# eora-ai/torchok

Hardware: AMD Instinct MI355X
Metric: images/sec (node) ResNet-50 224px bs256/GPU; step p50 ms (higher is better)
Workload: dtype bf16

## Files before the change

### include/tok.h

```cpp
#ifndef TOK_H_
#define TOK_H_

#include <stddef.h>
#include <stdint.h>

#ifdef __cplusplus
extern "C" {
#endif

typedef enum tok_status {
  TOK_OK = 0,
  TOK_ERR_INVALID = -1,
  TOK_ERR_LAUNCH = -2,
  TOK_ERR_WORKSPACE = -3
} tok_status;

typedef enum tok_dtype { TOK_F32 = 0, TOK_F16 = 1, TOK_BF16 = 2 } tok_dtype;

typedef struct tok_conv_desc {
  int32_t n, h, w, c;
  int32_t k;
  int32_t r, s;
  int32_t p, q;
  int32_t stride, pad;
  int32_t s_pad;
} tok_conv_desc;

const char* tok_last_error(void);
int tok_version(void);


int tok_nchw_to_nhwc_bf16(const void* src, int src_dtype, int n, int c, int h, int w,
                          void* dst, int c_pad, void* stream);
int tok_cast_f32_bf16(const float* src, void* dst, size_t count, void* stream);
int tok_cast_bf16_f32(const void* src, float* dst, float scale, size_t count, void* stream);
int tok_pack_weight_fwd(const float* src, int k, int r, int s, int c,
                        void* dst, int k_pad, int s_pad, int c_pad, void* stream);
int tok_pack_weight_dgrad(const float* src, int k, int r, int s, int c,
                          void* dst, int k_pad, int c_pad, void* stream);

int tok_pack_weight_both(const float* src, int k, int r, int s, int c, void* dst_fwd, int k_pad,
                         int s_pad, int c_pad, void* dst_dgrad, void* stream);

typedef struct tok_pack_item {
  const float* src;
  void* dst_fwd;
  void* dst_dgrad;
  int32_t k, r, s, c, k_pad, s_pad, c_pad;
  int32_t block_start;
} tok_pack_item;
int tok_pack_item_blocks(const tok_pack_item* item );
int tok_pack_weights_batched(const tok_pack_item* items_dev, int n_items, int total_blocks, void* stream);


int tok_conv_fwd_stat_rows(const tok_conv_desc* d);
int tok_conv_fwd(const tok_conv_desc* d, const void* x, const void* w, const float* bias,
                 void* y, float* stats, void* stream);
int tok_conv_dgrad(const tok_conv_desc* d, const void* dy, const void* w_dgrad, void* dx,
                   int accumulate, void* stream);
int tok_conv_dgrad_stat_rows(const tok_conv_desc* d);
int tok_conv_dgrad_bnstats(const tok_conv_desc* d, const void* dy, const void* w_dgrad, void* dx,
                           int accumulate, const void* bn_y, const uint8_t* bn_mask, float* partial,
                           void* stream);
int tok_bn_gram_finalize(const float* Z, const float* zsum, const float* w, int64_t count, int p, int k,
                         const float* gamma, const float* beta, float* running_mean, float* running_var,
                         int64_t* num_batches_tracked, float momentum, float eps, float* mean, float* rstd,
                         float* scale, float* shift, float* wz ,
                         void* stream);
int tok_conv_fwd_bn_apply(const tok_conv_desc* d, const void* x, const void* w, const float* scale, const float* shift,
                          const void* shortcut , int relu, void* out, uint8_t* mask ,
                          void* stream);
int tok_conv_dgrad_maskstore(const tok_conv_desc* d, const void* dy, const void* w_dgrad, void* dx, int accumulate,
                             const uint8_t* mask, float* partial, void* stream);
int tok_relu_mask_reduce(const void* dout, const uint8_t* mask, int64_t m, int c, void* dz, float* partial, void* stream);
int tok_bn3_bwd_prepare(const float* G, const float* w, const float* wz, const float* zsum, const float* partial, int rows,
                        int64_t count, int p, int k, const float* gamma, const float* mean, const float* rstd,
                        float* dgamma, float* dbeta, int param_accumulate, float* coef, float* dw, int dw_accumulate,
                        void* wa, void* wb, float* cvec, float* ws ,
                        void* stream);
size_t tok_bn3_bwd_prepare_ws_floats(int p, int k);
int tok_conv_dgrad_bias(const tok_conv_desc* d, const void* dy, const void* w_dgrad, const float* bias, void* dx,
                        int accumulate, const void* bn_y, const uint8_t* bn_mask, float* partial, void* stream);
int tok_subsample2_fwd(const void* x, int n, int h, int w, int c, void* out, void* stream);
int tok_subsample2_bwd(const void* dsub, int n, int h, int w, int c, void* dx, int accumulate, void* stream);
int tok_conv_dgrad_subacc_ok(const tok_conv_desc* d);
int tok_conv_dgrad_subacc(const tok_conv_desc* d, const void* dy, const void* w_dgrad, void* dx, const void* dsub,
                          const void* bn_y , const uint8_t* mask ,
                          float* partial , int mask_store, void* stream);
int tok_conv_dgrad2_ok(const tok_conv_desc* d1, const tok_conv_desc* d2);
int tok_conv_dgrad2(const tok_conv_desc* d1, const void* dy1, const void* w1_dgrad, const tok_conv_desc* d2, const void* dy2,
                    const void* w2_dgrad, const float* bias , void* dx, int accumulate,
                    const void* bn_y , const uint8_t* bn_mask , float* partial ,
                    void* stream);
size_t tok_conv_wgrad_ws_bytes(const tok_conv_desc* d);
int tok_conv_wgrad(const tok_conv_desc* d, const void* x, const void* dy, float* dw,
                   int k_real, int c_real, void* ws, size_t ws_bytes, int accumulate,
                   void* stream);
int tok_conv_wgrad_bias_ok(const tok_conv_desc* d);
size_t tok_conv_wgrad_bias_ws_bytes(const tok_conv_desc* d);
int tok_conv_wgrad_bias(const tok_conv_desc* d, const void* x, const void* dy, float* dw, int k_real, int c_real,
                        void* ws, size_t ws_bytes, int accumulate, float* dbias, int bias_accumulate, void* stream);


int tok_bn_finalize(const float* stats, int rows, int64_t count, int c, int c_real,
                    const float* gamma, const float* beta,
                    float* running_mean, float* running_var, int64_t* nbt,
                    float momentum, float eps,
                    float* mean, float* rstd, float* scale, float* shift, void* stream);
int tok_bn_eval_coeffs(const float* gamma, const float* beta, const float* running_mean,
                       const float* running_var, float eps, int c, int c_real,
                       float* scale, float* shift, void* stream);
int tok_bn_stats_rows(int64_t m, int c);
int tok_bn_stats(const void* y, int64_t m, int c, float* stats, void* stream);
int tok_bn_act_fwd(const void* y, const float* scale, const float* shift,
                   const void* shortcut, int relu, void* out, uint8_t* mask, int64_t m, int c,
                   void* stream);
void* tok_event_create(void);
int tok_event_destroy(void* ev);
int tok_next_launch_event(void* ev);
int tok_stream_wait_event(void* stream, void* ev);
int tok_bn_act_fwd_colsum_rows(int64_t m, int c);
int tok_bn_act_fwd_colsum(const void* y, const float* scale, const float* shift, const void* shortcut, int relu, void* out,
                          uint8_t* mask, int64_t m, int c, float* partial, void* stream);
int tok_bn_bwd_rows(int64_t m, int c);
int tok_bn_bwd_reduce(const void* dout, const void* y, const uint8_t* mask,
                      const float* scale, const float* shift,
                      const float* mean, const float* rstd, int relu,
                      int64_t m, int c, float* partial, void* stream);
int tok_bn_bwd_finalize(const float* partial, int rows, int64_t m, int c, int c_real,
                        const float* gamma, const float* mean, const float* rstd,
                        float* dgamma, float* dbeta, float* coef, int accumulate, int dzy_form,
                        void* stream);
int tok_bn_bwd_apply(const void* dout, const void* y, const uint8_t* mask,
                     const float* scale, const float* shift, const float* coef, int relu,
                     void* dy, void* dshortcut, int dshortcut_accumulate,
                     int64_t m, int c, void* stream);
int tok_bn_hswish_fwd(const void* y, const float* scale, const float* shift, void* out, int64_t m, int c, void* stream);
int tok_bn_hswish_bwd_reduce(const void* dout, const void* y, const float* scale, const float* shift, const float* mean,
                             const float* rstd, int64_t m, int c, float* partial, void* stream);
int tok_bn_hswish_bwd_apply(const void* dout, const void* y, const float* scale, const float* shift, const float* coef,
                            void* dy, int64_t m, int c, void* stream);
int tok_bn_relu6_fwd(const void* y, const float* scale, const float* shift, void* out, int64_t m, int c, void* stream);
int tok_bn_relu6_bwd_reduce(const void* dout, const void* y, const float* scale, const float* shift, const float* mean,
                            const float* rstd, int64_t m, int c, float* partial, void* stream);
int tok_bn_relu6_bwd_apply(const void* dout, const void* y, const float* scale, const float* shift, const float* coef,
                           void* dy, int64_t m, int c, void* stream);


int tok_maxpool3x3s2_fwd(const void* x, void* y, uint8_t* argmax, int n, int h, int w, int c,
                         void* stream);
int tok_maxpool3x3s2_bwd(const void* dy, const uint8_t* argmax, void* dx, int accumulate,
                         int n, int h, int w, int c, void* stream);
int tok_avgpool2x2_fwd(const void* x, void* y, int n, int h, int w, int c, void* stream);
int tok_avgpool2x2_bwd(const void* dy, void* dx, int accumulate, int n, int h, int w, int c, void* stream);
int tok_gap_fwd(const void* x, void* y, int n, int hw, int c, void* stream);
int tok_gap_bwd(const void* dy, void* dx, int accumulate, int n, int hw, int c, void* stream);
int tok_global_pool_fwd(const void* x, void* y, int* argmax, int n, int hw, int c, int ldy, int mode, void* stream);
int tok_global_pool_bwd(const void* dy, const int* argmax, void* dx, int accumulate, int n, int hw, int c, int ldy,
                        int mode, void* stream);

int tok_colsum(const void* dy, int64_t m, int n_pad, int n_real, float* out, int accumulate,
               void* stream);

#define TOK_CE_LOSS_FLOATS 2050
int tok_softmax_ce_fwd(const void* logits, const int64_t* target, int rows, int classes, int ld,
                       int64_t ignore_index, float* lse, float* row_loss,
                       float* loss , void* stream);
int tok_softmax_ce_bwd(const void* logits, const int64_t* target, const float* lse,
                       const float* loss, const float* gscale, int rows, int classes, int ld,
                       int64_t ignore_index, void* dlogits, void* stream);

int tok_softmax_ce_smooth_fwd(const void* logits, const int64_t* target, int rows, int classes, int ld,
                              int64_t ignore_index, float label_smoothing, float* lse, float* row_loss,
                              float* loss, void* stream);
int tok_softmax_ce_smooth_bwd(const void* logits, const int64_t* target, const float* lse, const float* loss,
                              const float* gscale, int rows, int classes, int ld, int64_t ignore_index,
                              float label_smoothing, void* dlogits, void* stream);

int tok_upsample_ce_serves(int classes, int ld);
int tok_upsample_ce_fwd(const void* low, int n, int hs, int ws, int classes, int ld, int hd, int wd, const int64_t* target,
// ... 278 lines not shown
```

### torchok_amd/_C.py

```python
import ctypes
import os
from ctypes import POINTER, Structure, c_char_p, c_float, c_int, c_int32, c_int64, c_size_t, c_void_p

_HERE = os.path.dirname(os.path.abspath(__file__))
LIB_PATH = os.environ.get('TOK_LIB') or os.path.join(_HERE, 'lib', 'libtok_gfx950.so')

TOK_F32, TOK_F16, TOK_BF16 = 0, 1, 2
TOK_CE_LOSS_FLOATS = 2050


class ConvDesc(Structure):
    _fields_ = [('n', c_int32), ('h', c_int32), ('w', c_int32), ('c', c_int32),
                ('k', c_int32), ('r', c_int32), ('s', c_int32),
                ('p', c_int32), ('q', c_int32),
                ('stride', c_int32), ('pad', c_int32), ('s_pad', c_int32)]


class PackItem(Structure):
    _fields_ = [('src', c_void_p), ('dst_fwd', c_void_p), ('dst_dgrad', c_void_p),
                ('k', c_int32), ('r', c_int32), ('s', c_int32), ('c', c_int32),
                ('k_pad', c_int32), ('s_pad', c_int32), ('c_pad', c_int32), ('block_start', c_int32)]


TOK_GRAD_CLIP_MAX_PARTIALS = 1024

_P = c_void_p
_PD = POINTER(ConvDesc)

PROTOTYPES = {
    'tok_last_error': (c_char_p, []),
    'tok_version': (c_int, []),
    'tok_nchw_to_nhwc_bf16': (c_int, [_P, c_int, c_int, c_int, c_int, c_int, _P, c_int, _P]),
    'tok_cast_f32_bf16': (c_int, [_P, _P, c_size_t, _P]),
    'tok_cast_bf16_f32': (c_int, [_P, _P, c_float, c_size_t, _P]),
    'tok_pack_weight_fwd': (c_int, [_P, c_int, c_int, c_int, c_int, _P, c_int, c_int, c_int, _P]),
    'tok_pack_weight_dgrad': (c_int, [_P, c_int, c_int, c_int, c_int, _P, c_int, c_int, _P]),
    'tok_pack_weight_both': (c_int, [_P, c_int, c_int, c_int, c_int, _P, c_int, c_int, c_int, _P, _P]),
    'tok_pack_item_blocks': (c_int, [POINTER(PackItem)]),
    'tok_pack_weights_batched': (c_int, [_P, c_int, c_int, _P]),
    'tok_conv_fwd_stat_rows': (c_int, [_PD]),
    'tok_conv_fwd': (c_int, [_PD, _P, _P, _P, _P, _P, _P]),
    'tok_conv_dgrad': (c_int, [_PD, _P, _P, _P, c_int, _P]),
    'tok_conv_dgrad_stat_rows': (c_int, [_PD]),
    'tok_conv_dgrad_bnstats': (c_int, [_PD, _P, _P, _P, c_int, _P, _P, _P, _P]),
    'tok_conv_wgrad_ws_bytes': (c_size_t, [_PD]),
    'tok_conv_wgrad': (c_int, [_PD, _P, _P, _P, c_int, c_int, _P, c_size_t, c_int, _P]),
    'tok_conv_wgrad_bias_ok': (c_int, [_PD]),
    'tok_conv_wgrad_bias_ws_bytes': (c_size_t, [_PD]),
    'tok_conv_wgrad_bias': (c_int, [_PD, _P, _P, _P, c_int, c_int, _P, c_size_t, c_int, _P, c_int, _P]),
    'tok_bn_finalize': (c_int, [_P, c_int, c_int64, c_int, c_int, _P, _P, _P, _P, _P, c_float, c_float,
                                _P, _P, _P, _P, _P]),
    'tok_bn_eval_coeffs': (c_int, [_P, _P, _P, _P, c_float, c_int, c_int, _P, _P, _P]),
    'tok_bn_stats_rows': (c_int, [c_int64, c_int]),
    'tok_bn_stats': (c_int, [_P, c_int64, c_int, _P, _P]),
    'tok_bn_act_fwd': (c_int, [_P, _P, _P, _P, c_int, _P, _P, c_int64, c_int, _P]),
    'tok_bn_act_fwd_colsum_rows': (c_int, [c_int64, c_int]),
    'tok_event_create': (_P, []),
    'tok_event_destroy': (c_int, [_P]),
    'tok_next_launch_event': (c_int, [_P]),
    'tok_stream_wait_event': (c_int, [_P, _P]),
    'tok_bn_act_fwd_colsum': (c_int, [_P, _P, _P, _P, c_int, _P, _P, c_int64, c_int, _P, _P]),
    'tok_bn_bwd_rows': (c_int, [c_int64, c_int]),
    'tok_bn_bwd_reduce': (c_int, [_P, _P, _P, _P, _P, _P, _P, c_int, c_int64, c_int, _P, _P]),
    'tok_bn_bwd_finalize': (c_int, [_P, c_int, c_int64, c_int, c_int, _P, _P, _P, _P, _P, _P, c_int, c_int, _P]),
    'tok_bn_bwd_apply': (c_int, [_P, _P, _P, _P, _P, _P, c_int, _P, _P, c_int, c_int64, c_int, _P]),
    'tok_bn_hswish_fwd': (c_int, [_P, _P, _P, _P, c_int64, c_int, _P]),
    'tok_bn_hswish_bwd_reduce': (c_int, [_P, _P, _P, _P, _P, _P, c_int64, c_int, _P, _P]),
    'tok_bn_hswish_bwd_apply': (c_int, [_P, _P, _P, _P, _P, _P, c_int64, c_int, _P]),
    'tok_bn_relu6_fwd': (c_int, [_P, _P, _P, _P, c_int64, c_int, _P]),
    'tok_bn_relu6_bwd_reduce': (c_int, [_P, _P, _P, _P, _P, _P, c_int64, c_int, _P, _P]),
    'tok_bn_relu6_bwd_apply': (c_int, [_P, _P, _P, _P, _P, _P, c_int64, c_int, _P]),
    'tok_maxpool3x3s2_fwd': (c_int, [_P, _P, _P, c_int, c_int, c_int, c_int, _P]),
    'tok_maxpool3x3s2_bwd': (c_int, [_P, _P, _P, c_int, c_int, c_int, c_int, c_int, _P]),
    'tok_avgpool2x2_fwd': (c_int, [_P, _P, c_int, c_int, c_int, c_int, _P]),
    'tok_avgpool2x2_bwd': (c_int, [_P, _P, c_int, c_int, c_int, c_int, c_int, _P]),
    'tok_gap_fwd': (c_int, [_P, _P, c_int, c_int, c_int, _P]),
    'tok_gap_bwd': (c_int, [_P, _P, c_int, c_int, c_int, c_int, _P]),
    'tok_global_pool_fwd': (c_int, [_P, _P, _P, c_int, c_int, c_int, c_int, c_int, _P]),
    'tok_global_pool_bwd': (c_int, [_P, _P, _P, c_int, c_int, c_int, c_int, c_int, c_int, _P]),
    'tok_colsum': (c_int, [_P, c_int64, c_int, c_int, _P, c_int, _P]),
    'tok_bn_gram_finalize': (c_int, [_P, _P, _P, c_int64, c_int, c_int, _P, _P, _P, _P, _P, c_float, c_float, _P, _P, _P, _P, _P, _P]),
    'tok_conv_fwd_bn_apply': (c_int, [POINTER(ConvDesc), _P, _P, _P, _P, _P, c_int, _P, _P, _P]),
    'tok_conv_dgrad_maskstore': (c_int, [POINTER(ConvDesc), _P, _P, _P, c_int, _P, _P, _P]),
    'tok_relu_mask_reduce': (c_int, [_P, _P, c_int64, c_int, _P, _P, _P]),
    'tok_bn3_bwd_prepare': (c_int, [_P, _P, _P, _P, _P, c_int, c_int64, c_int, c_int, _P, _P, _P, _P, _P, c_int, _P, _P, c_int,
                                    _P, _P, _P, _P, _P]),
    'tok_bn3_bwd_prepare_ws_floats': (c_size_t, [c_int, c_int]),
    'tok_conv_dgrad_bias': (c_int, [POINTER(ConvDesc), _P, _P, _P, _P, c_int, _P, _P, _P, _P]),
    'tok_conv_dgrad2_ok': (c_int, [POINTER(ConvDesc), POINTER(ConvDesc)]),
    'tok_conv_dgrad2': (c_int, [POINTER(ConvDesc), _P, _P, POINTER(ConvDesc), _P, _P, _P, _P, c_int, _P, _P, _P, _P]),
    'tok_subsample2_fwd': (c_int, [_P, c_int, c_int, c_int, c_int, _P, _P]),
    'tok_subsample2_bwd': (c_int, [_P, c_int, c_int, c_int, c_int, _P, c_int, _P]),
    'tok_conv_dgrad_subacc_ok': (c_int, [POINTER(ConvDesc)]),
    'tok_conv_dgrad_subacc': (c_int, [POINTER(ConvDesc), _P, _P, _P, _P, _P, _P, _P, c_int, _P]),
    'tok_softmax_ce_fwd': (c_int, [_P, _P, c_int, c_int, c_int, c_int64, _P, _P, _P, _P]),
    'tok_softmax_ce_bwd': (c_int, [_P, _P, _P, _P, _P, c_int, c_int, c_int, c_int64, _P, _P]),
    'tok_softmax_ce_smooth_fwd': (c_int, [_P, _P, c_int, c_int, c_int, c_int64, c_float, _P, _P, _P, _P]),
    'tok_softmax_ce_smooth_bwd': (c_int, [_P, _P, _P, _P, _P, c_int, c_int, c_int, c_int64, c_float, _P, _P]),
    'tok_upsample_ce_serves': (c_int, [c_int, c_int]),
    'tok_upsample_ce_fwd': (c_int, [_P, c_int, c_int, c_int, c_int, c_int, c_int, c_int, _P, c_int64, _P, _P, _P, _P]),
    'tok_upsample_ce_bwd': (c_int, [_P, c_int, c_int, c_int, c_int, c_int, c_int, c_int, _P, c_int64, _P, _P, _P, _P, c_int, _P]),
    'tok_dice_rows': (c_int, [c_int64]),
    'tok_dice_fwd': (c_int, [_P, _P, c_int64, c_int, c_int, c_int, c_float, c_float, c_int, _P, c_int, _P, _P, _P, _P]),
    'tok_dice_bwd': (c_int, [_P, _P, _P, _P, c_int64, c_int, c_int, c_int, _P, _P]),
    'tok_bce_logits_fwd': (c_int, [_P, _P, c_int64, c_int, c_int, c_float, c_int, _P, _P]),
    'tok_bce_logits_bwd': (c_int, [_P, _P, _P, _P, c_int64, c_int, c_int, c_float, c_int, _P, _P]),
    'tok_relevance_matrix_multilabel': (c_int, [_P, _P, c_int, c_int, c_int, _P, _P]),
    'tok_embed_reg_fwd': (c_int, [_P, c_int, c_int, c_int, c_int, _P, _P, _P]),
    'tok_embed_reg_bwd': (c_int, [_P, _P, _P, c_float, c_int, c_int, c_int, c_int, _P, _P]),
    'tok_regression_loss_fwd': (c_int, [_P, _P, c_int64, c_int, c_float, c_int, _P, _P]),
    'tok_regression_loss_bwd': (c_int, [_P, _P, _P, c_int64, c_int, c_float, c_int, _P, _P]),
    'tok_confusion_update': (c_int, [_P, _P, _P, c_int64, c_int, c_int, c_int64, _P, _P]),
    'tok_cls_stats_update': (c_int, [_P, _P, _P, c_int64, c_int, c_int, c_int64, _P, _P]),
    'tok_l2norm_fwd': (c_int, [_P, _P, _P, c_int, c_int, c_int, c_int, c_float, _P]),
    'tok_l2norm_bwd': (c_int, [_P, _P, _P, _P, c_int, c_int, c_int, c_int, c_int, _P]),
    'tok_arcface_margin_fwd': (c_int, [_P, _P, c_int, c_int, c_int, c_float, c_float, c_float, c_float, c_int, c_float, _P, _P]),
    'tok_arcface_margin_bwd': (c_int, [_P, _P, _P, c_int, c_int, c_int, c_float, c_float, c_float, c_float, c_int, c_float, _P, _P]),
    'tok_relevance_matrix': (c_int, [_P, _P, c_int, c_int, _P, _P]),
    'tok_contrastive_fwd': (c_int, [_P, _P, _P, c_int, c_int, c_int, c_int, c_float, _P, _P, _P, _P]),
    'tok_contrastive_bwd': (c_int, [_P, _P, _P, _P, _P, c_int, c_int, c_int, c_int, c_float, _P, _P, c_int, _P]),
    'tok_fuse_sum_relu_fwd': (c_int, [_P, c_int, _P, c_int, _P, c_int, _P, c_int, c_int, c_int, c_int, c_int, c_int, _P, _P, _P]),
    'tok_fuse_sum_affine_relu_fwd': (c_int, [_P, c_int, _P, _P, _P, c_int, _P, _P, _P, c_int, _P, _P, _P, c_int, _P, _P, c_int, c_int, c_int, c_int, c_int, _P, _P, _P]),
    'tok_fuse_sum_relu_bwd': (c_int, [_P, _P, c_int, c_int, c_int, c_int, c_int, _P, c_int, _P]),
    'tok_bilinear_fwd': (c_int, [_P, c_int, c_int, c_int, c_int, c_int, _P, c_int, c_int, c_int, c_int, _P]),
    'tok_bilinear_bwd': (c_int, [_P, c_int, c_int, c_int, c_int, c_int, _P, c_int, c_int, c_int, c_int, c_int, _P]),
    'tok_nearest_fwd': (c_int, [_P, c_int, c_int, c_int, c_int, c_int, _P, c_int, c_int, c_int, c_int, _P]),
    'tok_nearest_bwd': (c_int, [_P, c_int, c_int, c_int, c_int, c_int, _P, c_int, c_int, c_int, c_int, c_int, _P]),
    'tok_bilinear_bwd_multi': (c_int, [_P, c_int, c_int, c_int, c_int, _P, c_int, c_int, _P, c_int, c_int, _P, c_int, c_int, _P]),
    'tok_bilinear_sum_stats_rows': (c_int, [c_int, c_int, c_int, c_int]),
    'tok_bilinear_sum_stats': (c_int, [_P, _P, c_int, c_int, _P, c_int, c_int, _P, c_int, c_int, c_int, c_int, c_int, c_int, _P, _P, _P]),
    'tok_layernorm_fwd': (c_int, [_P, _P, _P, c_int, _P, _P, _P, _P, _P, c_int64, c_int, c_int, c_float, _P]),
    'tok_layernorm_bwd_rows': (c_int, [c_int64, c_int]),
    'tok_layernorm_bwd': (c_int, [_P, _P, _P, _P, _P, _P, c_int, _P, c_int, _P, c_int64, c_int, c_int, _P]),
    'tok_colsum_partial_rows': (c_int, [c_int64, c_int]),
    'tok_colsum_partial': (c_int, [_P, c_int64, c_int, _P, _P]),
    'tok_colsum_f32': (c_int, [_P, c_int64, c_int, _P, c_int, _P]),
    'tok_colsum_f32_pair': (c_int, [_P, _P, c_int64, c_int, _P, c_int, _P, c_int, _P]),
    'tok_act_fwd': (c_int, [c_int, _P, _P, c_size_t, _P]),
    'tok_act_bwd': (c_int, [c_int, _P, _P, _P, c_int, c_size_t, _P]),
    'tok_window_attn_fwd': (c_int, [_P, c_int, c_int, c_int, c_int, c_int, c_int, c_int, c_int, _P, _P, _P, _P, _P, _P]),
    'tok_window_attn_bwd_rows': (c_int, [c_int, c_int, c_int, c_int, c_int]),
    'tok_window_attn_bwd': (c_int, [_P, _P, c_int, c_int, c_int, c_int, c_int, c_int, c_int, c_int, _P, _P, _P, _P, _P,
                                    _P, _P, _P]),
    'tok_cpb_bias_fwd': (c_int, [_P, c_int, _P, c_int, c_int, _P, _P]),
    'tok_cpb_bias_bwd': (c_int, [_P, c_int, _P, c_int, _P, c_int, c_int, c_int, _P, _P]),
    'tok_patch_merge': (c_int, [_P, _P, c_int, c_int, c_int, c_int, c_int, _P]),
    'tok_ntxent_fwd': (c_int, [_P, c_int, c_int, c_int, c_float, _P, _P, _P, _P]),
    'tok_ntxent_bwd': (c_int, [_P, _P, _P, c_int, c_int, c_int, c_float, _P, _P]),
    'tok_triplet_fwd': (c_int, [_P, _P, _P, c_int, c_int, c_int, c_float, c_float, c_int, _P, _P, _P, _P]),
    'tok_triplet_bwd': (c_int, [_P, _P, _P, _P, _P, c_int, c_int, c_int, c_float, c_float, c_int, _P, _P, _P, _P]),
    'tok_bn_relu_maxpool_fwd': (c_int, [_P, _P, _P, c_int, c_int, c_int, c_int, _P, _P, _P, _P]),
    'tok_bn_pool_bwd_reduce_pooled': (c_int, [_P, _P, _P, _P, _P, c_int64, c_int, _P, _P]),
    'tok_bn_pool_bwd_reduce': (c_int, [_P, _P, _P, _P, _P, _P, _P, c_int, c_int, c_int, c_int, _P, _P]),
    'tok_bn_pool_bwd_apply': (c_int, [_P, _P, _P, _P, _P, _P, c_int, c_int, c_int, c_int, _P, _P]),
    'tok_conv_fwd_act': (c_int, [_PD, _P, _P, _P, _P, _P, c_int, _P]),
    'tok_conv_dgrad_act': (c_int, [_PD, _P, _P, _P, c_int, _P, _P]),
    'tok_mlp_serves': (c_int, [c_int64, c_int, c_int]),
    'tok_mlp_fwd': (c_int, [_P, _P, _P, _P, _P, _P, _P, _P, c_int64, c_int, c_int, _P]),
    'tok_mlp_bwd_dx': (c_int, [_P, _P, _P, _P, _P, c_int, _P, c_int64, c_int, c_int, _P]),
    'tok_chan_gram': (c_int, [_P, c_int, _P, c_int, c_int, c_int, c_int, c_float, c_int, _P, _P, _P]),
    'tok_chan_apply': (c_int, [_P, c_int, _P, c_int, c_float, c_int, c_int, c_int, _P, c_int, _P]),
    'tok_scale_rows_add': (c_int, [_P, _P, _P, c_int, _P, c_int, c_int64, c_int, _P]),
    'tok_pix_class_matmul': (c_int, [_P, c_int, _P, c_int, c_int, c_int, c_int, c_int, c_float, _P, _P]),
    'tok_class_pix_expand': (c_int, [_P, _P, c_int, c_int, c_int, c_int, c_int, c_float, _P, c_int, c_int, _P]),
    'tok_weighted_pool_chunks': (c_int, [c_int]),
    'tok_weighted_pool': (c_int, [_P, _P, c_int, c_int, c_int, c_int, c_int, c_float, _P, _P, c_int, c_int, _P]),
    'tok_softmax_rows_f32': (c_int, [_P, c_int64, c_int, _P, _P]),
    'tok_softmax_rows_bwd_f32': (c_int, [_P, _P, c_int64, c_int, _P, _P]),
    'tok_softmax_cols_fwd': (c_int, [_P, c_int, c_int, c_int, c_int, c_float, _P, _P]),
    'tok_softmax_cols_bwd': (c_int, [_P, _P, c_int, c_int, c_int, c_float, _P, c_int, c_int, _P]),
    'tok_channel_scale': (c_int, [_P, _P, _P, c_int, c_int, c_int, c_int, c_int, _P]),
    'tok_dwconv3x3': (c_int, [_P, _P, _P, _P, c_int, c_int, c_int, c_int, c_int, c_int, c_int, _P]),
    'tok_dwconv3x3_wgrad_blocks': (c_int, [c_int, c_int]),
    'tok_dwconv3x3_wgrad': (c_int, [_P, _P, c_int, c_int, c_int, c_int, c_int, _P, _P, _P, c_int, _P]),
    'tok_dwconv_rows': (c_int, [c_int, c_int, c_int, c_int, c_int, c_int]),
    'tok_dwconv_fwd': (c_int, [_P, _P, c_int, c_int, c_int, c_int, c_int, c_int, c_int, _P, _P, _P]),
    'tok_dwconv_dgrad': (c_int, [_P, _P, c_int, c_int, c_int, c_int, c_int, c_int, c_int, _P, c_int, _P]),
# ... 94 lines not shown
```

### torchok_amd/csrc/conv_igemm.hip

```cpp
#include "conv_common.h"
#include "pw_gemm.h"
#include <stdlib.h>

namespace {

constexpr int BK = 64;
#ifdef TOK_NO_FRAG_ASM
constexpr bool FRAG_ASM = false;
#else
constexpr bool FRAG_ASM = true;
#endif
#ifdef TOK_NO_DMA
constexpr bool DMA_ENABLED = false;
#else
constexpr bool DMA_ENABLED = true;
#endif

__device__ __forceinline__ int fw_swz(int n) {
  return ((0x78 >> (((n >> 3) & 3) << 1)) & 3) | (((n >> 1) & 1) << 2);
}

template <int BM, int BN, int IN_DIV, bool C4, int PWM>
__global__ __launch_bounds__(256, (BN == 64 && PWM != 4) ? 3 : 2) void conv_igemm_kernel(ConvArgs a) {
  constexpr bool PW = PWM != 0;
// ... 268 lines not shown
    if constexpr (DMA && FRAG_ASM) {
      const uint32_t Ab = lds_base + buf * TILE_BYTES, Wb = Ab + BM * BK * 2;
      u32x4 wf[2][4], af[2][MT];
#pragma unroll
      for (int kk = 0; kk < 2; ++kk) {
        const int s = sl + 4 * kk;
#pragma unroll
        for (int t = 0; t < 4; ++t) wf[kk][t] = lds_read16(Wb + (wrow0 + (t >> 1) * 32 + (t & 1) * 4) * 128 + ((s ^ wswz) << 4));
#pragma unroll
        for (int mt = 0; mt < MT; ++mt) af[kk][mt] = lds_read16(Ab + (arow0 + mt * 16) * 128 + ((s ^ aswz) << 4));
      }
      asm volatile("s_waitcnt lgkmcnt(%0)" ::"n"(4 + MT) : "memory");
      __builtin_amdgcn_sched_barrier(0);
#pragma unroll
      for (int t = 0; t < 4; ++t)
#pragma unroll
        for (int mt = 0; mt < MT; ++mt)
          acc[t][mt] = __builtin_amdgcn_mfma_f32_16x16x32_bf16(__builtin_bit_cast(bf16x8, wf[0][t]),
                                                               __builtin_bit_cast(bf16x8, af[0][mt]), acc[t][mt], 0, 0, 0);
      __builtin_amdgcn_sched_barrier(0);
      asm volatile("s_waitcnt lgkmcnt(0)" ::: "memory");
      __builtin_amdgcn_sched_barrier(0);
#pragma unroll
      for (int t = 0; t < 4; ++t)
#pragma unroll
        for (int mt = 0; mt < MT; ++mt)
          acc[t][mt] = __builtin_amdgcn_mfma_f32_16x16x32_bf16(__builtin_bit_cast(bf16x8, wf[1][t]),
                                                               __builtin_bit_cast(bf16x8, af[1][mt]), acc[t][mt], 0, 0, 0);
      return;
    }
    const char* Ab = smem + buf * TILE_BYTES;
    const char* Wb = Ab + BM * BK * 2;
#pragma unroll
    for (int kk = 0; kk < 2; ++kk) {
      bf16x8 wf[4], af[MT];
      const int s = sl + 4 * kk;
#pragma unroll
      for (int t = 0; t < 4; ++t)
        wf[t] = *reinterpret_cast<const bf16x8*>(Wb + (wrow0 + (t >> 1) * 32 + (t & 1) * 4) * 128 +
                                                 ((s ^ wswz) << 4));
#pragma unroll
      for (int mt = 0; mt < MT; ++mt)
        af[mt] = *reinterpret_cast<const bf16x8*>(Ab + (arow0 + mt * 16) * 128 + ((s ^ aswz) << 4));
#pragma unroll
      for (int t = 0; t < 4; ++t)
#pragma unroll
        for (int mt = 0; mt < MT; ++mt)
          acc[t][mt] = __builtin_amdgcn_mfma_f32_16x16x32_bf16(wf[t], af[mt], acc[t][mt], 0, 0, 0);
    }
  };

  auto epilogue = [&](const Ctx& ctx) {
    const int nb = ctx.n0 + wn * 64 + sl * 8;
    if (a.bias != nullptr) {
#pragma unroll
      for (int c = 0; c < 16; ++c) {
        const int n = nb + (c >> 3) * 32 + (c & 7);
        const float bv = n < a.K ? a.bias[n] : 0.f;
#pragma unroll
        for (int mt = 0; mt < MT; ++mt) acc[c >> 2][mt][c & 3] += bv;
      }
    }
    size_t opix_[MT];
    bool rowok_[MT];
#pragma unroll
    for (int mt = 0; mt < MT; ++mt) {
      const int ml = ctx.m0 + arow0 + mt * 16;
      if (IN_DIV == 2) {
        rowok_[mt] = ml < a.cls_M[ctx.cls];
        const uint32_t mm = rowok_[mt] ? ml : 0;
        const uint32_t b = fdiv(mm, a.cls_fd_hw[ctx.cls]);
        const uint32_t rem = mm - b * a.cls_hw[ctx.cls];
        const uint32_t h2 = fdiv(rem, a.cls_fd_w[ctx.cls]);
        const uint32_t w2 = rem - h2 * a.cls_nw[ctx.cls];
        opix_[mt] = ((size_t)b * a.P + (2 * h2 + (ctx.cls >> 1))) * a.Q + (2 * w2 + (ctx.cls & 1));
      } else {
        rowok_[mt] = ml < a.M;
        opix_[mt] = (size_t)ml;
      }
    }
    bf16x8 pre_old[MT][2], pre_y[MT][2];
    unsigned pre_bits[MT][2];
    const bool want_old = a.accumulate != 0;
    const bool want_y = a.stats != nullptr && !a.mask_store && a.bn_y != nullptr;
    const bool want_bits = a.bn_mask != nullptr && (a.mask_store || want_y);
    constexpr bool PRE = !BNEP && !ACT && !C4;
    if (PRE) {
#pragma unroll
      for (int mt = 0; mt < MT; ++mt)
#pragma unroll
        for (int half = 0; half < 2; ++half) {
          const bool ok = rowok_[mt] && nb + half * 32 + 8 <= a.K;
          const size_t eoff = opix_[mt] * a.K + nb + half * 32;
          pre_old[mt][half] = (ok && want_old) ? ldg16(a.y + eoff) : zero8();
          pre_y[mt][half] = (ok && want_y) ? ldg16(a.bn_y + eoff) : zero8();
          pre_bits[mt][half] = (ok && want_bits) ? (unsigned)a.bn_mask[eoff >> 3] : 0xffu;
        }
    }
#pragma unroll
    for (int mt = 0; mt < MT; ++mt) {
      const size_t opix = opix_[mt];
      const bool rowok = rowok_[mt];
      if (rowok) {
        bf16* yp = a.y + opix * a.K + nb;
#pragma unroll
        for (int half = 0; half < 2; ++half) {
          if (nb + half * 32 + 8 <= a.K) {
            bf16x8 o;
            float v[8];
#pragma unroll
            for (int e = 0; e < 8; ++e) v[e] = acc[half * 2 + (e >> 2)][mt][e & 3];
            if (a.accumulate) {
              const bf16x8 old = PRE ? pre_old[mt][half] : ldg16(yp + half * 32);
#pragma unroll
              for (int e = 0; e < 8; ++e) v[e] += bf2f(old[e]);
            }
#pragma unroll
            for (int e = 0; e < 8; ++e) o[e] = f2bf(v[e]);
            if (ACT) {
              const size_t eoff = opix * a.K + nb + half * 32;
              if (a.act_x != nullptr) {
                const bf16x8 hx = ldg16(a.act_x + eoff);
#pragma unroll
                for (int e = 0; e < 8; ++e) {
                  const float f = bf2f(hx[e]);
                  const float dd = a.act == 0 ? (f > 0.f ? 1.f : 0.f) : gelu_d(f);
                  o[e] = f2bf(bf2f(o[e]) * dd);
                }
              }
              if (a.y2 != nullptr) {
                bf16x8 o2;
#pragma unroll
                for (int e = 0; e < 8; ++e) {
                  const float f = bf2f(o[e]);
                  o2[e] = f2bf(a.act == 0 ? fmaxf(f, 0.f) : gelu_f(f));
                }
                stg16(a.y2 + eoff, o2);
              }
            }
            if (BNEP) {
              const int n0 = nb + half * 32;
              const size_t eoff = opix * a.K + n0;
              bf16x8 sv = zero8();
              if (a.ep_short != nullptr)
                sv = *reinterpret_cast<const bf16x8*>(sbase + s_rd * S_BYTES + (arow0 + mt * 16) * 128 +
                                                      (((sl + 4 * half) ^ aswz) << 4));
              unsigned bits = 0;
#pragma unroll
              for (int e = 0; e < 8; ++e) {
                float z = fmaf(v[e], esc[half * 8 + e], esh[half * 8 + e]) + bf2f(sv[e]);
                if (a.ep_relu) z = fmaxf(z, 0.f);
                o[e] = f2bf(z);
                bits |= (bf2f(o[e]) > 0.f ? 1u : 0u) << e;
              }
              if (a.ep_mask != nullptr) a.ep_mask[eoff >> 3] = (uint8_t)bits;
            }
            if (a.mask_store) {
              const unsigned bits = PRE ? pre_bits[mt][half] : (unsigned)a.bn_mask[(opix * a.K + nb + half * 32) >> 3];
#pragma unroll
              for (int e = 0; e < 8; ++e) {
                if (!((bits >> e) & 1u)) o[e] = (bf16)0.f;
                s1[half * 8 + e] += bf2f(o[e]);
              }
            }
            if (NTS) __builtin_nontemporal_store(o, reinterpret_cast<bf16x8*>(yp + half * 32));
            else stg16(yp + half * 32, o);
            if (a.stats != nullptr && !a.mask_store) {
              if (a.bn_y != nullptr) {
                const size_t eoff = opix * a.K + nb + half * 32;
                const bf16x8 yv = PRE ? pre_y[mt][half] : ldg16(a.bn_y + eoff);
                const unsigned bits = PRE ? pre_bits[mt][half] : (a.bn_mask != nullptr ? (unsigned)a.bn_mask[eoff >> 3] : 0xffu);
#pragma unroll
                for (int e = 0; e < 8; ++e) {
                  const float dz = ((bits >> e) & 1u) ? bf2f(o[e]) : 0.f;
                  s1[half * 8 + e] += dz;
                  s2[half * 8 + e] = fmaf(dz, bf2f(yv[e]), s2[half * 8 + e]);
                }
              } else {
#pragma unroll
                for (int e = 0; e < 8; ++e) {
                  const float r = bf2f(o[e]);
                  s1[half * 8 + e] += r;
                  s2[half * 8 + e] = fmaf(r, r, s2[half * 8 + e]);
                }
              }
            }
          }
        }
      }
    }
  };

  int it = xcd * S8 + jm;
  bool any = it < a.gridM;
  Ctx cur = {0, bn_fixed * BN, 0, 0};
  bool cur_has = false;
  if (any) {
    cur = setup(it);
    seek();
    cur_has = kt < a.KT;
    if (cur_has) { load_tile(0); store_tile(0); }
  }
  if (DMA) asm volatile("s_waitcnt vmcnt(0)" ::: "memory");
  __syncthreads();
  zero_acc();
  int buf = 0;
#ifdef TOK_TIMING
  unsigned long long tacc[6] = {0, 0, 0, 0, 0, 0};
  const unsigned long long tk0 = __builtin_amdgcn_s_memtime();
#endif
  while (any) {
    bool tile_done, nxt_has, any_next = true;
    Ctx nxt = cur;
    if (cur_has) { advance(); ++kt; seek(); }
    if (kt < a.KT) {
      tile_done = false;
      nxt_has = true;
    } else {
      tile_done = true;
      it += sweep;
      any_next = it < a.gridM;
      nxt_has = false;
      if (any_next) {
        nxt = setup(it);
        seek();
        nxt_has = kt < a.KT;
      }
    }
#ifdef TOK_TIMING
    const unsigned long long t0 = __builtin_amdgcn_s_memtime();
#endif
    ld_on = nxt_has;
    load_tile(buf ^ 1);
#ifdef TOK_TIMING
    const unsigned long long t1 = __builtin_amdgcn_s_memtime();
#endif
    if (cur_has) compute(buf);
#ifdef TOK_TIMING
    __builtin_amdgcn_sched_barrier(0);
    const unsigned long long t2 = __builtin_amdgcn_s_memtime();
#endif
    if (tile_done) {
      epilogue(cur);
      zero_acc();
      if (BNEP) s_rd ^= 1;
// ... 368 lines not shown
                            const float* bias, void* y, float* stats, void* stream) {
  return conv_fwd_impl(d, x, w, bias, y, stats, stream);
}

extern "C" int tok_conv_fwd_act(const tok_conv_desc* d, const void* x, const void* w, const float* bias, void* y,
                                void* y_act, int kind, void* stream) {
  TOK_CHECK_ARG(y_act != nullptr && (kind == 0 || kind == 1), "tok_conv_fwd_act: y_act and kind 0 (ReLU) / 1 (GELU)");
  return conv_fwd_impl(d, x, w, bias, y, nullptr, stream, y_act, kind);
}

extern "C" int tok_conv_dgrad_act(const tok_conv_desc* d, const void* dy, const void* w_dgrad, const void* act_x, int kind,
                                  void* dx, void* stream) {
  TOK_CHECK_ARG(act_x != nullptr && (kind == 0 || kind == 1), "tok_conv_dgrad_act: act_x and kind 0 (ReLU) / 1 (GELU)");
  DgradEpilogue ep = {}; ep.act_x = act_x; ep.act = kind;
  return dgrad_impl(d, dy, w_dgrad, dx, ep, stream, "tok_conv_dgrad_act");
}

extern "C" int tok_conv_dgrad(const tok_conv_desc* d, const void* dy, const void* w_dgrad, void* dx,
                              int accumulate, void* stream) {
  DgradEpilogue ep = {}; ep.accumulate = accumulate;
  return dgrad_impl(d, dy, w_dgrad, dx, ep, stream, "tok_conv_dgrad");
}

extern "C" int tok_conv_dgrad_stat_rows(const tok_conv_desc* d) {
  if (check_desc(d, "tok_conv_dgrad_stat_rows")) return TOK_ERR_INVALID;
  ConvArgs a = {};
  if (dgrad_fill(d, a)) return TOK_ERR_INVALID;
  return route_dgrad(d, a, ConvMode{}).stat_rows;
}

extern "C" int tok_conv_dgrad_bnstats(const tok_conv_desc* d, const void* dy, const void* w_dgrad, void* dx,
                                      int accumulate, const void* bn_y, const uint8_t* bn_mask,
                                      float* partial, void* stream) {
  TOK_CHECK_ARG(bn_y && partial, "tok_conv_dgrad_bnstats: bn_y / partial must not be null");
  DgradEpilogue ep = {}; ep.accumulate = accumulate; ep.bn_y = bn_y; ep.bn_mask = bn_mask; ep.partial = partial;
  return dgrad_impl(d, dy, w_dgrad, dx, ep, stream, "tok_conv_dgrad_bnstats");
}



extern "C" int tok_conv_fwd_bn_apply(const tok_conv_desc* d, const void* x, const void* w, const float* scale,
                                     const float* shift, const void* shortcut, int relu, void* out, uint8_t* mask,
                                     void* stream) {
  TOK_CHECK_ARG(d && scale && shift && out, "tok_conv_fwd_bn_apply: null pointer");
  TOK_CHECK_ARG(d->r == 1 && d->s == 1 && d->stride == 1 && d->pad == 0 && d->c % 8 == 0,
                "tok_conv_fwd_bn_apply: 1x1 / stride 1 / no padding layers only");
  const BnEpilogue ep = {scale, shift, shortcut, mask, relu};
  return conv_fwd_impl(d, x, w, nullptr, out, nullptr, stream, nullptr, 0, &ep);
}

extern "C" int tok_conv_dgrad_maskstore(const tok_conv_desc* d, const void* dy, const void* w_dgrad, void* dx,
                                        int accumulate, const uint8_t* mask, float* partial, void* stream) {
  TOK_CHECK_ARG(mask && partial, "tok_conv_dgrad_maskstore: mask / partial must not be null");
  DgradEpilogue ep = {}; ep.accumulate = accumulate; ep.bn_mask = mask; ep.partial = partial; ep.mask_store = 1;
  return dgrad_impl(d, dy, w_dgrad, dx, ep, stream, "tok_conv_dgrad_maskstore");
}

extern "C" int tok_conv_dgrad_bias(const tok_conv_desc* d, const void* dy, const void* w_dgrad, const float* bias, void* dx,
                                   int accumulate, const void* bn_y, const uint8_t* bn_mask, float* partial, void* stream) {
  TOK_CHECK_ARG((bn_y == nullptr) == (partial == nullptr), "tok_conv_dgrad_bias: bn_y and partial go together");
  DgradEpilogue ep = {}; ep.accumulate = accumulate; ep.bn_y = bn_y; ep.bn_mask = bn_mask; ep.partial = partial; ep.bias = bias;
  return dgrad_impl(d, dy, w_dgrad, dx, ep, stream, "tok_conv_dgrad_bias");
}


extern "C" int tok_conv_dgrad_subacc_ok(const tok_conv_desc* d) {
  if (check_desc(d, "tok_conv_dgrad_subacc_ok")) return 0;
  if (!(d->r == 1 && d->s == 1 && d->stride == 1 && d->pad == 0 && d->c % 8 == 0)) return 0;
  ConvArgs a = {};
  if (dgrad_fill(d, a)) return 0;
  return route_dgrad(d, a, ConvMode{false, false,  true, false}).kernel == K_RING ? 1 : 0;
}

extern "C" int tok_conv_dgrad_subacc(const tok_conv_desc* d, const void* dy, const void* w_dgrad, void* dx, const void* dsub,
                                     const void* bn_y, const uint8_t* mask, float* partial, int mask_store, void* stream) {
  TOK_CHECK_ARG(dsub != nullptr, "tok_conv_dgrad_subacc: dsub must not be null");
  TOK_CHECK_ARG(!mask_store || (mask && partial && !bn_y), "tok_conv_dgrad_subacc: mask_store needs mask + partial, no bn_y");
  TOK_CHECK_ARG(mask_store || ((bn_y == nullptr) == (partial == nullptr)), "tok_conv_dgrad_subacc: bn_y and partial go together");
  DgradEpilogue ep = {}; ep.bn_y = bn_y; ep.bn_mask = mask; ep.partial = partial; ep.mask_store = mask_store; ep.sub = dsub;
  return dgrad_impl(d, dy, w_dgrad, dx, ep, stream, "tok_conv_dgrad_subacc");
}


namespace {
bool dgrad2_route(const tok_conv_desc* d1, const tok_conv_desc* d2, ConvRoute* r) {
  if (d1 == nullptr || d2 == nullptr) return false;
  for (const tok_conv_desc* d : {d1, d2})
    if (!(d->r == 1 && d->s == 1 && d->stride == 1 && d->pad == 0 && d->k % 8 == 0 && d->c % 64 == 0)) return false;
  if (d1->n != d2->n || d1->h != d2->h || d1->w != d2->w || d1->c != d2->c) return false;
  const long long rows = (long long)d1->n * d1->h * d1->w;
  ConvArgs g = {};
  g.M = (int)rows; g.C = g.Ktot = d2->k; g.K = d2->c; g.R = g.S = g.stride = 1;
  g.gridM = tok_cdiv(rows, 128);
  *r = route_gemm(g, true, pick_bn(d2->c, d2->k), ConvMode{});
  return r->kernel == K_RING && r->bn_tile == 64;
}
}

extern "C" int tok_conv_dgrad2_ok(const tok_conv_desc* d1, const tok_conv_desc* d2) { ConvRoute r; return dgrad2_route(d1, d2, &r) ? 1 : 0; }

extern "C" int tok_conv_dgrad2(const tok_conv_desc* d1, const void* dy1, const void* w1_dgrad, const tok_conv_desc* d2,
                               const void* dy2, const void* w2_dgrad, const float* bias, void* dx, int accumulate,
                               const void* bn_y, const uint8_t* bn_mask, float* partial, void* stream) {
  ConvRoute r;
  TOK_CHECK_ARG(dgrad2_route(d1, d2, &r), "tok_conv_dgrad2: layers not served (ask tok_conv_dgrad2_ok)");
  TOK_CHECK_ARG(dy1 && w1_dgrad && dy2 && w2_dgrad && dx, "tok_conv_dgrad2: null pointer");
  TOK_CHECK_ARG((bn_y == nullptr) == (partial == nullptr), "tok_conv_dgrad2: bn_y and partial go together");
  PwArgs p = {};
  p.x = (const bf16*)dy1; p.w = (const bf16*)w1_dgrad; p.C = d1->k;
  p.x2 = (const bf16*)dy2; p.w2 = (const bf16*)w2_dgrad; p.C2 = d2->k;
  p.y = (bf16*)dx; p.bias = bias; p.stats = partial;
  p.M = d1->n * d1->h * d1->w; p.N = d1->c;
  p.gridM = r.gridM; p.gridN = r.gridN; p.stat_rows = r.stat_rows;
  p.e1 = accumulate ? (const bf16*)dx : nullptr;
  p.accumulate = accumulate;
  p.e2 = (const bf16*)bn_y; p.mask_in = bn_mask;
  const int rc = pw_ring_launch(p, 64, r.grid, tok_stream(stream));
  if (rc != 0) { tok_set_error("tok_conv_dgrad2: ring kernel refused the launch (%d)", rc); return TOK_ERR_INVALID; }
  TOK_CHECK_LAUNCH("tok_conv_dgrad2");
  return TOK_OK;
}
```

### torchok_amd/csrc/conv_wgrad.hip

```cpp
#include "tok_common.h"
#include "conv_common.h"
#include <type_traits>
#include <stdlib.h>

namespace {

struct WgradArgs {
  const bf16* x;
  const bf16* dy;
  float* ws;
  int H, W, C, K, R, S, P, Q, stride, pad;
  int M, PQ, HW, Ktot;
  int tilesN, tilesK, splitM, mchunk;
  uint32_t x_bytes, dy_bytes;
  uint32_t pq_mul, pq_shift, q_mul, q_shift;
  float* cs;
  int cs_cols;
  int adv_q, adv_p;
  size_t cs_stride, ws_stride;
};

__device__ __forceinline__ uint32_t magic_div(uint32_t n, uint32_t mul, uint32_t shift) {
  return (uint32_t)(((uint64_t)__umulhi(n, mul) + n) >> shift);
}
void make_magic(uint32_t d, uint32_t& mul, uint32_t& shift) {
  mul = 0; shift = 0;
  if (d <= 1) return;
  uint32_t l = 0;
  while ((1ull << l) < d) ++l;
  mul = (uint32_t)((((1ull << 32) * ((1ull << l) - d)) / d) + 1);
  shift = l;
}

typedef __attribute__((address_space(3))) bf16x4 lds_bf16x4;

__device__ __forceinline__ u32x2 tr_read_asm(uint32_t lds_addr) {
  u32x2 v;
  asm volatile("ds_read_b64_tr_b16 %0, %1" : "=v"(v) : "v"(lds_addr));
  return v;
}

__device__ __forceinline__ bf16x4 tr_read(const char* p) {
  return __builtin_amdgcn_ds_read_tr16_b64_v4bf16((lds_bf16x4*)(p));
}

template <int TN, int TK, bool C4, int MS, bool PWK>
__global__ __launch_bounds__(256) void conv_wgrad_kernel(WgradArgs a) {
  constexpr int CN = TN / 8, CK = TK / 8;
  constexpr int RPY = 256 / CN, RPX = 256 / CK;
  constexpr int YP = MS / RPY, XP = MS / RPX;
  constexpr bool DMA = !C4;
  constexpr int YS = DMA ? TN * 2 : (TN + 16) * 2, XS = DMA ? TK * 2 : (TK + 16) * 2;
  constexpr int YBYTES = MS * YS, XBYTES = MS * XS;
  constexpr int SWY = CN / 2 - 1, SWX = CK / 2 - 1;
  constexpr int NT = TN / 32, KTL = TK / 32;

  extern __shared__ __attribute__((aligned(16))) char smem[];

  const int tid = threadIdx.x;
  const int lane = tid & 63;
  const int wv = tid >> 6;
  const int wn2 = wv & 1, wk2 = wv >> 1;

  const int ntile = a.tilesN * a.tilesK;
  const int id = tok_xcd_remap(blockIdx.x, ntile * a.splitM);
  const int split = id / ntile;
  const int t = id - split * ntile;
  const int tn = t / a.tilesK;
  const int tk = t - tn * a.tilesK;

  const int mstart = split * a.mchunk;
  const int mend = min(a.M, mstart + a.mchunk);
  const int steps = (mend - mstart + MS - 1) / MS;

  const int ycol = tid % CN, yrow = tid / CN;
  const int xcol = tid % CK, xrow = tid / CK;
  const int ylog = DMA ? (ycol ^ ((yrow & SWY) << 1)) : ycol;
  const int xlog = DMA ? (xcol ^ ((xrow & SWX) << 1)) : xcol;
  const int wave_u = __builtin_amdgcn_readfirstlane(tid >> 6);
  const int yn = tn * TN + ylog * 8;
  const bool yn_ok = yn < a.K;

  const int k0 = tk * TK + xlog * 8;
  int kr, ks, kc0;
  if (C4) { kr = k0 >> 5; ks = (k0 & 31) >> 2; kc0 = 0; }
  else { const int tap = k0 / a.C; kc0 = k0 - tap * a.C; kr = tap / a.S; ks = tap - kr * a.S; }
  const bool k_ok = kr < a.R;
  constexpr bool pointwise = PWK;

  int xm[XP];
#pragma unroll
  for (int i = 0; i < XP; ++i) xm[i] = mstart + xrow + i * RPX;
  int ym = mstart + yrow;

  bf16x8 ry[YP], rx[XP];

  const __amdgpu_buffer_rsrc_t ysrd = __builtin_amdgcn_make_buffer_rsrc((void*)a.dy, 0, a.dy_bytes, 0x00020000);
  const __amdgpu_buffer_rsrc_t xsrd = __builtin_amdgcn_make_buffer_rsrc((void*)a.x, 0, a.x_bytes, 0x00020000);
  typedef __attribute__((address_space(3))) void lds_void;
  auto load_tile = [&](int dbuf) {
    char* Ydst = smem + dbuf * (YBYTES + XBYTES) + wave_u * 1024;
    char* Xdst = smem + dbuf * (YBYTES + XBYTES) + YBYTES + wave_u * 1024;
// ... 87 lines not shown
    const char* Xb = Yb + YBYTES;
    if constexpr (true) {
      constexpr int HALVES = MS / 32;
      const uint32_t Yl = lds_base + (st & 1) * (YBYTES + XBYTES), Xl = Yl + YBYTES;
      u32x2 ya[HALVES][NT][2], xb[HALVES][KTL][2];
#pragma unroll
      for (int ks = 0; ks < HALVES; ++ks) {
#pragma unroll
        for (int i = 0; i < NT; ++i) {
          ya[ks][i][0] = tr_read_asm(Yl + (rrow + ks * 32) * YS + ycolb(i));
          ya[ks][i][1] = tr_read_asm(Yl + (rrow + ks * 32 + 16) * YS + ycolb(i));
        }
#pragma unroll
        for (int j = 0; j < KTL; ++j) {
          xb[ks][j][0] = tr_read_asm(Xl + (rrow + ks * 32) * XS + xcolb(j));
          xb[ks][j][1] = tr_read_asm(Xl + (rrow + ks * 32 + 16) * XS + xcolb(j));
        }
      }
#pragma unroll
      for (int ks = 0; ks < HALVES; ++ks) {
        __builtin_amdgcn_sched_barrier(0);
        if (ks + 1 < HALVES) asm volatile("s_waitcnt lgkmcnt(%0)" ::"n"(2 * (NT + KTL) > 15 ? 15 : 2 * (NT + KTL)) : "memory");
        else asm volatile("s_waitcnt lgkmcnt(0)" ::: "memory");
        __builtin_amdgcn_sched_barrier(0);
#pragma unroll
        for (int i = 0; i < NT; ++i) {
          const bf16x8 af = __builtin_bit_cast(bf16x8, (u32x4){ya[ks][i][0][0], ya[ks][i][0][1], ya[ks][i][1][0], ya[ks][i][1][1]});
#pragma unroll
          for (int j = 0; j < KTL; ++j) {
            const bf16x8 bfr = __builtin_bit_cast(bf16x8, (u32x4){xb[ks][j][0][0], xb[ks][j][0][1], xb[ks][j][1][0], xb[ks][j][1][1]});
            acc[i][j] = __builtin_amdgcn_mfma_f32_16x16x32_bf16(af, bfr, acc[i][j], 0, 0, 0);
          }
        }
      }
      __builtin_amdgcn_sched_barrier(0);
      if (DMA) asm volatile("s_waitcnt vmcnt(0)" ::: "memory");
      else store_tile((st + 1) & 1);
      __syncthreads();
      continue;
    }
#pragma unroll
    for (int ks = 0; ks < MS / 32; ++ks) {
      bf16x8 af[NT], bfr[KTL];
#pragma unroll
      for (int i = 0; i < NT; ++i) {
        const bf16x4 lo = tr_read(Yb + (rrow + ks * 32) * YS + ycolb(i));
        const bf16x4 hi = tr_read(Yb + (rrow + ks * 32 + 16) * YS + ycolb(i));
#pragma unroll
        for (int e = 0; e < 4; ++e) { af[i][e] = lo[e]; af[i][4 + e] = hi[e]; }
      }
#pragma unroll
      for (int j = 0; j < KTL; ++j) {
        const bf16x4 lo = tr_read(Xb + (rrow + ks * 32) * XS + xcolb(j));
        const bf16x4 hi = tr_read(Xb + (rrow + ks * 32 + 16) * XS + xcolb(j));
#pragma unroll
        for (int e = 0; e < 4; ++e) { bfr[j][e] = lo[e]; bfr[j][4 + e] = hi[e]; }
      }
#pragma unroll
      for (int i = 0; i < NT; ++i)
#pragma unroll
        for (int j = 0; j < KTL; ++j)
          acc[i][j] = __builtin_amdgcn_mfma_f32_16x16x32_bf16(af[i], bfr[j], acc[i][j], 0, 0, 0);
    }
    store_tile((st + 1) & 1);
    __syncthreads();
  }

  float* out = a.ws + (size_t)split * a.K * a.Ktot;
#pragma unroll
  for (int i = 0; i < NT; ++i) {
#pragma unroll
    for (int j = 0; j < KTL; ++j) {
      const int kcol = tk * TK + wk2 * (TK / 2) + j * 16 + li;
#pragma unroll
      for (int r = 0; r < 4; ++r) {
        const int n = tn * TN + wn2 * (TN / 2) + i * 16 + g * 4 + r;
        if (n < a.K && kcol < a.Ktot) out[(size_t)n * a.Ktot + kcol] = acc[i][j][r];
      }
    }
  }
}


template <int TN, int TK, int WK>
__global__ __launch_bounds__(128 * WK, WK == 4 ? 1 : 0) void conv_wgrad_ring_kernel(WgradArgs a) {
  constexpr int MS = 32, NST = 3, NTHR = 128 * WK;
  constexpr int CN = TN / 8, CK = TK / 8;
  constexpr int RPY = NTHR / CN, RPX = NTHR / CK;
  constexpr int YP = MS / RPY, XP = MS / RPX;
  static_assert(YP >= 1 && XP >= 1 && MS % RPY == 0 && MS % RPX == 0, "tile too narrow for the thread count");
  constexpr int LOADS = YP + XP;
  constexpr int YS = TN * 2, XS = TK * 2;
  constexpr int YBYTES = MS * YS, XBYTES = MS * XS, STAGE = YBYTES + XBYTES;
  constexpr int SWY = (CN / 2 - 1) < (RPY - 1) ? (CN / 2 - 1) : (RPY - 1);
  constexpr int SWX = (CK / 2 - 1) < (RPX - 1) ? (CK / 2 - 1) : (RPX - 1);
  constexpr int NT = TN / 32, KTL = TK / (16 * WK);

  extern __shared__ __attribute__((aligned(16))) char smem[];

  const int tid = threadIdx.x;
  const int lane = tid & 63;
  const int wv = tid >> 6;
  const int wn2 = wv & 1, wk = wv >> 1;

  const int ntile = a.tilesN * a.tilesK;
  const int id = tok_xcd_remap(blockIdx.x, ntile * a.splitM);
  const int split = id / ntile;
  const int t = id - split * ntile;
  const int tn = t / a.tilesK;
  const int tk = t - tn * a.tilesK;

  const int mstart = split * a.mchunk;
  const int mend = min(a.M, mstart + a.mchunk);
  const int steps = (mend - mstart + MS - 1) / MS;

  const int ycol = tid % CN, yrow = tid / CN;
  const int xcol = tid % CK, xrow = tid / CK;
  const int ylog = ycol ^ ((yrow & SWY) << 1);
  const int xlog = xcol ^ ((xrow & SWX) << 1);
  const int wave_u = __builtin_amdgcn_readfirstlane(tid >> 6);
  const int yn = tn * TN + ylog * 8;
  const bool yn_ok = yn < a.K;

  int kc0;
  bool k_ok;
  if constexpr (WK == 2) {
    const int k0 = tk * TK + xlog * 8;
    const int tap = k0 / a.C;
    kc0 = k0 - tap * a.C;
    const int kr = tap / a.S;
    k_ok = kr < a.R;
  } else {
    kc0 = tk * TK + xlog * 8;
    k_ok = kc0 < a.C;
  }

  int xm[XP];
#pragma unroll
  for (int i = 0; i < XP; ++i) xm[i] = mstart + xrow + i * RPX;
  int ym = mstart + yrow;

  const __amdgpu_buffer_rsrc_t ysrd = __builtin_amdgcn_make_buffer_rsrc((void*)a.dy, 0, a.dy_bytes, 0x00020000);
  const __amdgpu_buffer_rsrc_t xsrd = __builtin_amdgcn_make_buffer_rsrc((void*)a.x, 0, a.x_bytes, 0x00020000);
  typedef __attribute__((address_space(3))) void lds_void;

  auto issue = [&](int dbuf) {
    char* Ydst = smem + dbuf * STAGE + wave_u * 1024;
    char* Xdst = smem + dbuf * STAGE + YBYTES + wave_u * 1024;
#pragma unroll
    for (int i = 0; i < YP; ++i) {
      const int m = ym + i * RPY;
      uint32_t off = (yn_ok && m < mend) ? (uint32_t)(m * a.K + yn) * 2u : 0xFFFFFFF0u;
      asm volatile("" : "+v"(off));
      __builtin_amdgcn_raw_ptr_buffer_load_lds(ysrd, (lds_void*)(Ydst + i * RPY * YS), 16, off, 0, 0, 0);
    }
    ym += MS;
#pragma unroll
    for (int i = 0; i < XP; ++i) {
      uint32_t off = (k_ok && xm[i] < mend) ? (uint32_t)(xm[i] * a.C + kc0) * 2u : 0xFFFFFFF0u;
      asm volatile("" : "+v"(off));
      __builtin_amdgcn_raw_ptr_buffer_load_lds(xsrd, (lds_void*)(Xdst + i * RPX * XS), 16, off, 0, 0, 0);
      xm[i] += MS;
    }
  };

  const int g = lane >> 4, li = lane & 15;
  const int rrow = 4 * g + (li >> 2);
  const int yswz = ((rrow & SWY) << 1) << 4, xswz = ((rrow & SWX) << 1) << 4;
  auto ycolb = [&](int i) { return ((wn2 * (TN / 2) + i * 16 + (li & 3) * 4) * 2) ^ yswz; };
  auto xcolb = [&](int j) { return ((wk * (TK / WK) + j * 16 + (li & 3) * 4) * 2) ^ xswz; };

  f32x4 acc[NT][KTL];
#pragma unroll
  for (int i = 0; i < NT; ++i)
#pragma unroll
    for (int j = 0; j < KTL; ++j) acc[i][j] = (f32x4){0.f, 0.f, 0.f, 0.f};

  const bool do_cs = a.cs != nullptr && tk == 0 && wk == 0;
  f32x4 csacc[NT];
#pragma unroll
  for (int i = 0; i < NT; ++i) csacc[i] = (f32x4){0.f, 0.f, 0.f, 0.f};
  const bf16 one_b = (bf16)1.0f;
  const bf16x8 ones = {one_b, one_b, one_b, one_b, one_b, one_b, one_b, one_b};

  typedef __attribute__((address_space(3))) char lds_char;
  const uint32_t lds_base = (uint32_t)(size_t)(lds_char*)smem;
  issue(0);
  issue(1);
  int cur = 0, nxt = 2;
  for (int st = 0; st < steps; ++st) {
    asm volatile("s_waitcnt vmcnt(%0) lgkmcnt(0)" ::"n"(LOADS) : "memory");
    __builtin_amdgcn_s_barrier();
    issue(nxt);
    const uint32_t Yb = lds_base + cur * STAGE;
    const uint32_t Xb = Yb + YBYTES;
    u32x2 ya[NT][2], xb[KTL][2];
    bf16x8 af[NT], bfr[KTL];
    if constexpr (WK == 2) {
#pragma unroll
      for (int i = 0; i < NT; ++i) {
        ya[i][0] = tr_read_asm(Yb + rrow * YS + ycolb(i));
        ya[i][1] = tr_read_asm(Yb + (rrow + 16) * YS + ycolb(i));
      }
#pragma unroll
      for (int j = 0; j < KTL; ++j) {
        xb[j][0] = tr_read_asm(Xb + rrow * XS + xcolb(j));
        xb[j][1] = tr_read_asm(Xb + (rrow + 16) * XS + xcolb(j));
      }
      asm volatile("s_waitcnt lgkmcnt(0)" ::: "memory");
      __builtin_amdgcn_sched_barrier(0);
#pragma unroll
      for (int i = 0; i < NT; ++i) af[i] = __builtin_bit_cast(bf16x8, (u32x4){ya[i][0][0], ya[i][0][1], ya[i][1][0], ya[i][1][1]});
#pragma unroll
      for (int j = 0; j < KTL; ++j) bfr[j] = __builtin_bit_cast(bf16x8, (u32x4){xb[j][0][0], xb[j][0][1], xb[j][1][0], xb[j][1][1]});
#pragma unroll
      for (int i = 0; i < NT; ++i)
#pragma unroll
        for (int j = 0; j < KTL; ++j)
          acc[i][j] = __builtin_amdgcn_mfma_f32_16x16x32_bf16(af[i], bfr[j], acc[i][j], 0, 0, 0);
    } else {
#pragma unroll
      for (int j = 0; j < KTL; ++j) {
        xb[j][0] = tr_read_asm(Xb + rrow * XS + xcolb(j));
        xb[j][1] = tr_read_asm(Xb + (rrow + 16) * XS + xcolb(j));
      }
#pragma unroll
      for (int i = 0; i < NT; ++i) {
        ya[i][0] = tr_read_asm(Yb + rrow * YS + ycolb(i));
        ya[i][1] = tr_read_asm(Yb + (rrow + 16) * YS + ycolb(i));
      }
      asm volatile("s_waitcnt lgkmcnt(8)" ::: "memory");
      __builtin_amdgcn_sched_barrier(0);
#pragma unroll
      for (int j = 0; j < KTL; ++j) bfr[j] = __builtin_bit_cast(bf16x8, (u32x4){xb[j][0][0], xb[j][0][1], xb[j][1][0], xb[j][1][1]});
#pragma unroll
      for (int i = 0; i < NT / 2; ++i) {
        af[i] = __builtin_bit_cast(bf16x8, (u32x4){ya[i][0][0], ya[i][0][1], ya[i][1][0], ya[i][1][1]});
#pragma unroll
        for (int j = 0; j < KTL; ++j) acc[i][j] = __builtin_amdgcn_mfma_f32_16x16x32_bf16(af[i], bfr[j], acc[i][j], 0, 0, 0);
      }
      asm volatile("s_waitcnt lgkmcnt(0)" ::: "memory");
      __builtin_amdgcn_sched_barrier(0);
#pragma unroll
      for (int i = NT / 2; i < NT; ++i) {
        af[i] = __builtin_bit_cast(bf16x8, (u32x4){ya[i][0][0], ya[i][0][1], ya[i][1][0], ya[i][1][1]});
#pragma unroll
        for (int j = 0; j < KTL; ++j) acc[i][j] = __builtin_amdgcn_mfma_f32_16x16x32_bf16(af[i], bfr[j], acc[i][j], 0, 0, 0);
      }
    }
    if (do_cs) {
#pragma unroll
      for (int i = 0; i < NT; ++i) csacc[i] = __builtin_amdgcn_mfma_f32_16x16x32_bf16(af[i], ones, csacc[i], 0, 0, 0);
    }
    cur = cur == NST - 1 ? 0 : cur + 1;
    nxt = nxt == NST - 1 ? 0 : nxt + 1;
  }
  asm volatile("s_waitcnt vmcnt(0)" ::: "memory");

  if (do_cs && li == 0) {
#pragma unroll
    for (int i = 0; i < NT; ++i)
#pragma unroll
      for (int r = 0; r < 4; ++r) {
        const int n = tn * TN + wn2 * (TN / 2) + i * 16 + g * 4 + r;
        if (n < a.cs_cols) a.cs[(size_t)split * a.cs_stride + n] = csacc[i][r];
      }
  }

  float* out = a.ws + (size_t)split * a.ws_stride;
#pragma unroll
  for (int i = 0; i < NT; ++i) {
#pragma unroll
    for (int j = 0; j < KTL; ++j) {
      const int kcol = tk * TK + wk * (TK / WK) + j * 16 + li;
#pragma unroll
      for (int r = 0; r < 4; ++r) {
        const int n = tn * TN + wn2 * (TN / 2) + i * 16 + g * 4 + r;
        if (n < a.K && kcol < a.Ktot) out[(size_t)n * a.Ktot + kcol] = acc[i][j][r];
      }
    }
  }
}


template <int DUMMY>
__global__ __launch_bounds__(256, 1) void conv_wgrad_taps_kernel(WgradArgs a) {
  constexpr int MS = 32, NST = 3, TN = 64, TC = 64, TAPS = 9;
  constexpr int TILE = MS * 128;
  constexpr int STAGE = (1 + TAPS) * TILE;
  constexpr int LOADS = 1 + TAPS;
  constexpr int NT = 4, KTL = 9;

  extern __shared__ __attribute__((aligned(16))) char smem[];

  const int tid = threadIdx.x;
  const int lane = tid & 63;
  const int wv = __builtin_amdgcn_readfirstlane(tid >> 6);

  const int tilesC = a.tilesK;
  const int ntile = a.tilesN * tilesC;
  const int id = tok_xcd_remap(blockIdx.x, ntile * a.splitM);
  const int split = id / ntile;
  const int t = id - split * ntile;
  const int tn = t / tilesC;
  const int ct = t - tn * tilesC;

  const int mstart = split * a.mchunk;
  const int mend = min(a.M, mstart + a.mchunk);
  const int steps = (mend - mstart + MS - 1) / MS;

  const int row = tid >> 3, cc = tid & 7;
  const int clog = cc ^ ((row & 3) << 1);
  const int yn = tn * TN + clog * 8;
  const bool yn_ok = yn < a.K;
  const int cx = ct * TC + clog * 8;
  const bool cx_ok = cx < a.C;

  const __amdgpu_buffer_rsrc_t ysrd = __builtin_amdgcn_make_buffer_rsrc((void*)a.dy, 0, a.dy_bytes, 0x00020000);
  const __amdgpu_buffer_rsrc_t xsrd = __builtin_amdgcn_make_buffer_rsrc((void*)a.x, 0, a.x_bytes, 0x00020000);
  typedef __attribute__((address_space(3))) void lds_void;

  int mcur = mstart + row;
  auto issue = [&](int slot) {
    char* base = smem + slot * STAGE + wv * 1024;
    const int m = mcur;
    const bool mok = m < mend;
    {
      uint32_t off = (uint32_t)(m * a.K + yn) * 2u;
      asm volatile("" : "+v"(off));
      off = (mok && yn_ok) ? off : 0xFFFFFFF0u;
      asm volatile("" : "+v"(off));
      __builtin_amdgcn_raw_ptr_buffer_load_lds(ysrd, (lds_void*)base, 16, off, 0, 0, 0);
    }
    const uint32_t mm = (uint32_t)min(m, a.M - 1);
    const uint32_t b = magic_div(mm, a.pq_mul, a.pq_shift);
    const uint32_t rem = mm - b * (uint32_t)a.PQ;
    const uint32_t pp = magic_div(rem, a.q_mul, a.q_shift);
    const int h0 = (int)pp * a.stride - a.pad;
    const int w0 = (int)(rem - pp * (uint32_t)a.Q) * a.stride - a.pad;
    const int xbase = (((int)b * a.H + h0) * a.W + w0) * a.C + cx;
    const bool live = mok && cx_ok;
    bool hok[3], wok[3];
#pragma unroll
    for (int k = 0; k < 3; ++k) {
      hok[k] = live && (unsigned)(h0 + k) < (unsigned)a.H;
      wok[k] = (unsigned)(w0 + k) < (unsigned)a.W;
    }
#pragma unroll
    for (int tap = 0; tap < TAPS; ++tap) {
      const int kr = tap / 3, ks = tap - kr * 3;
      uint32_t off = (uint32_t)(xbase + (kr * a.W + ks) * a.C) * 2u;
      asm volatile("" : "+v"(off));
      off = (hok[kr] && wok[ks]) ? off : 0xFFFFFFF0u;
      asm volatile("" : "+v"(off));
      __builtin_amdgcn_raw_ptr_buffer_load_lds(xsrd, (lds_void*)(base + (1 + tap) * TILE), 16, off, 0, 0, 0);
    }
    mcur += MS;
  };

  const int g = lane >> 4, li = lane & 15;
  const int rrow = 4 * g + (li >> 2);
// ... 324 lines not shown
      const int su = sp + 16 * u;
      v[u] = reinterpret_cast<const float4*>(ws + (size_t)(su < splitM ? su : splitM - 1) * stride)[i];
    }
#pragma unroll
    for (int u = 0; u < U; ++u) {
      if (sp + 16 * u < splitM) { t.x += v[u].x; t.y += v[u].y; t.z += v[u].z; t.w += v[u].w; }
    }
  }
}

__global__ __launch_bounds__(256) void wgrad_reduce_flat_kernel(const float* __restrict__ ws, float* __restrict__ dw,
                                                                int splitM, size_t slab, int accumulate, size_t stride,
                                                                float* __restrict__ extra, int extra_n, int extra_pad,
                                                                int extra_acc) {
  __shared__ float4 red[16][16];
  const int col = threadIdx.x & 15, row = threadIdx.x >> 4;
  const size_t m4 = slab >> 2;
  const size_t n4 = m4 + (extra != nullptr ? (size_t)(extra_pad >> 2) : 0);
  for (size_t base = (size_t)blockIdx.x * 16; base < n4; base += (size_t)gridDim.x * 16) {
    const size_t i = base + col;
    float4 t = {0.f, 0.f, 0.f, 0.f};
    if (i < n4) {
      if (splitM > 64) reduce_slabs<8>(ws, stride, i, row, splitM, t);
      else if (splitM > 32) reduce_slabs<4>(ws, stride, i, row, splitM, t);
      else if (splitM > 16) reduce_slabs<2>(ws, stride, i, row, splitM, t);
      else if (row < splitM) {
        const float4 v = reinterpret_cast<const float4*>(ws + (size_t)row * stride)[i];
        t.x += v.x; t.y += v.y; t.z += v.z; t.w += v.w;
      }
    }
    red[row][col] = t;
    __syncthreads();
    for (int s_ = 8; s_ > 0; s_ >>= 1) {
      if (row < s_) {
        const float4 o = red[row + s_][col];
        float4 m = red[row][col];
        m.x += o.x; m.y += o.y; m.z += o.z; m.w += o.w;
        red[row][col] = m;
      }
      __syncthreads();
    }
    if (row == 0 && i < m4) {
      float4 r = red[0][col];
      if (accumulate) {
        const float4 o = reinterpret_cast<const float4*>(dw)[i];
        r.x += o.x; r.y += o.y; r.z += o.z; r.w += o.w;
      }
      reinterpret_cast<float4*>(dw)[i] = r;
    } else if (row == 0 && i < n4) {
      const float4 r = red[0][col];
      const float rv[4] = {r.x, r.y, r.z, r.w};
      const int e0 = (int)(i - m4) * 4;
#pragma unroll
      for (int e = 0; e < 4; ++e)
        if (e0 + e < extra_n) extra[e0 + e] = extra_acc ? extra[e0 + e] + rv[e] : rv[e];
    }
    __syncthreads();
  }
}

enum Route {
  kStem,
  kWindow,
  kTaps,
  kRing,
  kTwoBuf
};

struct Plan {
  Route route;
  int TN, TK, tilesN, tilesK, splitM, mchunk, MS;
};

static void split_m(Plan& p, long long M, int target, int tiles, int MS, int cap) {
  long long split = (target + tiles - 1) / tiles;
  const long long max_split = (M + 8 * MS - 1) / (8 * MS);
  if (split > max_split) split = max_split;
  if (split > cap) split = cap;
  if (split < 1) split = 1;
  long long chunk = (M + split - 1) / split;
  chunk = (chunk + MS - 1) / MS * MS;
  p.mchunk = (int)chunk;
  p.splitM = (int)((M + chunk - 1) / chunk);
}

Plan make_plan(const tok_conv_desc* d) {
  Plan p;
  const int Ktot = d->r * d->s_pad * d->c;
  const long long M = (long long)d->n * d->p * d->q;
  const bool is3x3 = d->r == 3 && d->s == 3 && d->s_pad == 3;
  const bool pointwise = d->r == 1 && d->s == 1 && d->stride == 1 && d->pad == 0;
  const bool same3 = is3x3 && d->stride == 1 && d->pad == 1 &&
                     (unsigned long long)d->n * d->h * d->w * d->c * 2 < 0x40000000ull &&
                     (unsigned long long)d->n * d->p * d->q * d->k * 2 < 0x40000000ull;
  const bool w64 = d->c % 64 == 0 && d->k % 64 == 0;
  const bool w48 = !w64 && d->c % 48 == 0 && d->k % 48 == 0 && same3;
  if (d->c != 4 && (w64 || w48) && is3x3) {
    static const int target = tok_env_int("TOK_WGRAD_TAPS_WGS", 256);
    p.route = same3 && d->p == d->h && d->q == d->w ? kWindow : kTaps;
    p.TN = w64 ? 64 : 48; p.TK = p.TN; p.MS = 32;
    p.tilesN = tok_cdiv(d->k, p.TN);
    p.tilesK = tok_cdiv(d->c, p.TN);
    split_m(p, M, target, p.tilesN * p.tilesK, 32, 512);
    return p;
  }
  if (d->c != 4 && pointwise) {
    p.route = kRing; p.MS = 32;
    if (d->k <= 64) { p.TN = 64; p.TK = Ktot >= 256 ? 256 : (Ktot >= 128 ? 128 : 64); }
    else if (Ktot <= 64) { p.TK = 64; p.TN = d->k >= 256 ? 256 : 128; }
    else { p.TN = 128; p.TK = 128; }
    static const int big = tok_env_int("TOK_WGRAD_256", 1);
    if (big && d->k >= 256 && Ktot >= 256 && M >= (big >= 2 ? 8192 : 200000) &&
        (long long)tok_cdiv(d->k, 256) * tok_cdiv(Ktot, 256) * 65536 * 2 <= (long long)d->k * Ktot * 3) {
      p.TN = 256; p.TK = 256;
    }
    p.tilesN = tok_cdiv(d->k, p.TN);
    p.tilesK = tok_cdiv(Ktot, p.TK);
    const int stage = 32 * (p.TN + p.TK) * 2;
    const int per_cu = (160 * 1024) / (3 * stage);
    static const int ring_target = tok_env_int("TOK_WGRAD_WGS", 0), long_target = tok_env_int("TOK_WGRAD_WGS_LONG", 0);
    const int target = (long_target > 0 && M >= 100000) ? long_target
                       : ring_target > 0 ? ring_target : 256 * (per_cu > 2 ? 2 : per_cu);
    split_m(p, M, target, p.tilesN * p.tilesK, 32, 512);
    return p;
  }
  p.route = stem_wgrad_serves(d) ? kStem : kTwoBuf;
  p.TN = d->k >= 128 ? 128 : 64;
  p.TK = Ktot >= 128 ? 128 : 64;
  p.tilesN = tok_cdiv(d->k, p.TN);
  p.tilesK = tok_cdiv(Ktot, p.TK);
  const int tiles = p.tilesN * p.tilesK;
  p.MS = (M >= 100000 && p.TN == 128 && p.TK == 128) ? 64 : 32;
  static const int target = tok_env_int("TOK_WGRAD_2BUF_WGS", 1024);
  split_m(p, M, target, tiles, p.MS, (d->c == 4 && tiles <= 2) ? 512 : 256);
  return p;
}

template <int TN, int TK, int WK>
void launch_ring(const WgradArgs& a, hipStream_t st) {
  constexpr int smem = 3 * 32 * (TN + TK) * 2;
  tok_launch_lds<&conv_wgrad_ring_kernel<TN, TK, WK>>(smem, dim3(a.tilesN * a.tilesK * a.splitM), dim3(128 * WK), smem, st, a);
}

template <int TN, int TK, bool C4, int MS>
void launch_2buf_ms(const WgradArgs& a, hipStream_t st) {
  constexpr int smem = 2 * MS * ((TN + 16) * 2 + (TK + 16) * 2);
  const dim3 grid(a.tilesN * a.tilesK * a.splitM);
  if constexpr (!C4) {
    if (a.R == 1 && a.S == 1 && a.stride == 1 && a.pad == 0) {
      tok_launch_lds<&conv_wgrad_kernel<TN, TK, C4, MS, true>>(smem, grid, dim3(256), smem, st, a);
      return;
    }
  }
  tok_launch_lds<&conv_wgrad_kernel<TN, TK, C4, MS, false>>(smem, grid, dim3(256), smem, st, a);
}

template <int TN, int TK, bool C4>
void launch_2buf(const WgradArgs& a, hipStream_t st, int ms) {
  if (ms == 64) launch_2buf_ms<TN, TK, C4, 64>(a, st);
  else launch_2buf_ms<TN, TK, C4, 32>(a, st);
}

template <bool C4>
void launch_2buf_tile(const Plan& p, const WgradArgs& a, hipStream_t st) {
  if (p.TN == 128 && p.TK == 128) launch_2buf<128, 128, C4>(a, st, p.MS);
  else if (p.TN == 128) launch_2buf<128, 64, C4>(a, st, p.MS);
  else if (p.TK == 128) launch_2buf<64, 128, C4>(a, st, p.MS);
  else launch_2buf<64, 64, C4>(a, st, p.MS);
}

}

extern "C" size_t tok_conv_wgrad_ws_bytes(const tok_conv_desc* d) {
  if (d == nullptr) return 0;
  const Plan p = make_plan(d);
  return (size_t)p.splitM * d->k * d->r * d->s_pad * d->c * sizeof(float);
}

extern "C" int tok_conv_wgrad_bias_ok(const tok_conv_desc* d) {
  if (d == nullptr || d->c == 4) return 0;
  return make_plan(d).route == kRing ? 1 : 0;
}

extern "C" size_t tok_conv_wgrad_bias_ws_bytes(const tok_conv_desc* d) {
  if (d == nullptr) return 0;
  const Plan p = make_plan(d);
  return tok_conv_wgrad_ws_bytes(d) + (size_t)p.splitM * d->k * sizeof(float);
}

namespace {
int wgrad_impl(const tok_conv_desc* d, const void* x, const void* dy, float* dw, int k_real, int c_real, void* ws, size_t ws_bytes,
               int accumulate, float* dbias, int bias_accumulate, void* stream);
}

extern "C" int tok_conv_wgrad(const tok_conv_desc* d, const void* x, const void* dy, float* dw,
                              int k_real, int c_real, void* ws, size_t ws_bytes, int accumulate,
                              void* stream) {
  return wgrad_impl(d, x, dy, dw, k_real, c_real, ws, ws_bytes, accumulate, nullptr, 0, stream);
}

extern "C" int tok_conv_wgrad_bias(const tok_conv_desc* d, const void* x, const void* dy, float* dw, int k_real, int c_real,
                                   void* ws, size_t ws_bytes, int accumulate, float* dbias, int bias_accumulate, void* stream) {
  TOK_CHECK_ARG(dbias != nullptr, "tok_conv_wgrad_bias: dbias must not be null");
  TOK_CHECK_ARG(tok_conv_wgrad_bias_ok(d), "tok_conv_wgrad_bias: layer not served (ask tok_conv_wgrad_bias_ok)");
  return wgrad_impl(d, x, dy, dw, k_real, c_real, ws, ws_bytes, accumulate, dbias, bias_accumulate, stream);
}

namespace {
int wgrad_impl(const tok_conv_desc* d, const void* x, const void* dy, float* dw, int k_real, int c_real, void* ws, size_t ws_bytes,
               int accumulate, float* dbias, int bias_accumulate, void* stream) {
  TOK_CHECK_ARG(d && x && dy && dw && ws, "tok_conv_wgrad: null pointer");
  if (tok_dbg_skip(16)) return TOK_OK;
  TOK_CHECK_ARG(d->k % 8 == 0 && (d->c % 8 == 0 || d->c == 4), "tok_conv_wgrad: bad channel padding");
  TOK_CHECK_ARG(k_real <= d->k && c_real <= d->c, "tok_conv_wgrad: real dims exceed padded dims");
  TOK_CHECK_ARG(d->c == 4 ? d->s_pad == 8 : d->s_pad == d->s, "tok_conv_wgrad: bad s_pad");
  const Plan p = make_plan(d);
  const size_t need = dbias ? tok_conv_wgrad_bias_ws_bytes(d) : tok_conv_wgrad_ws_bytes(d);
  if (ws_bytes < need) {
    tok_set_error("tok_conv_wgrad: workspace %zu < %zu bytes", ws_bytes, need);
    return TOK_ERR_WORKSPACE;
  }
  const bool flat = (k_real == d->k) && (c_real == d->c) && (d->s_pad == d->s) &&
                    (((size_t)d->k * d->r * d->s * d->c) % 4 == 0) && (((uintptr_t)dw & 15) == 0);
  const bool direct = flat && p.splitM == 1 && !accumulate;
  WgradArgs a;
  a.x = (const bf16*)x; a.dy = (const bf16*)dy; a.ws = direct ? dw : (float*)ws;
  a.H = d->h; a.W = d->w; a.C = d->c; a.K = d->k; a.R = d->r; a.S = d->s_pad; a.P = d->p; a.Q = d->q;
  a.stride = d->stride; a.pad = d->pad;
  a.M = d->n * d->p * d->q; a.PQ = d->p * d->q; a.HW = d->h * d->w;
  make_magic((uint32_t)a.PQ, a.pq_mul, a.pq_shift);
  make_magic((uint32_t)d->q, a.q_mul, a.q_shift);
  a.adv_q = 32 % d->q; a.adv_p = (32 / d->q) % d->p;
  a.Ktot = d->r * d->s_pad * d->c;
  a.tilesN = p.tilesN; a.tilesK = p.tilesK; a.splitM = p.splitM; a.mchunk = p.mchunk;
  const size_t slab_f = (size_t)d->k * d->r * d->s_pad * d->c;
  const int cs_pad = (k_real + 3) / 4 * 4;
  const bool cs_inline = dbias != nullptr && flat && !direct;
  a.ws_stride = cs_inline ? slab_f + cs_pad : slab_f;
  a.cs = dbias ? (cs_inline ? (float*)ws + slab_f : (float*)((char*)ws + tok_conv_wgrad_ws_bytes(d))) : nullptr;
  a.cs_stride = cs_inline ? a.ws_stride : (size_t)k_real;
  a.cs_cols = k_real;
  {
    const unsigned long long xb = (unsigned long long)d->n * d->h * d->w * d->c * 2;
    const unsigned long long yb = (unsigned long long)a.M * d->k * 2;
    TOK_CHECK_ARG(xb < 0xFFFFFFF0ull && yb < 0xFFFFFFF0ull, "tok_conv_wgrad: tensors of 4 GiB or more are not supported");
    a.x_bytes = (uint32_t)xb; a.dy_bytes = (uint32_t)yb;
  }
  hipStream_t st = tok_stream(stream);
  const dim3 grid(a.tilesN * a.tilesK * a.splitM);
  switch (p.route) {
    case kStem:
      stem_wgrad_launch(d, x, dy, a.ws, p.splitM, st);
      break;
    case kWindow: {
      constexpr int smem = 3 * (32 * 128 + 128 * 128);
      if (p.TN == 48) tok_launch_lds<&conv_wgrad_winp_kernel<3, 3, 7>>(smem, grid, dim3(256), smem, st, a);
      else tok_launch_lds<&conv_wgrad_winp_kernel<4, 3, 9>>(smem, grid, dim3(256), smem, st, a);
      break;
    }
    case kTaps: {
      constexpr int smem = 3 * 10 * 32 * 128;
      tok_launch_lds<&conv_wgrad_taps_kernel<0>>(smem, grid, dim3(256), smem, st, a);
      break;
    }
    case kRing:
      if (p.TN == 256 && p.TK == 256) launch_ring<256, 256, 4>(a, st);
      else if (p.TN == 64 && p.TK == 64) launch_ring<64, 64, 2>(a, st);
      else if (p.TN == 64 && p.TK == 128) launch_ring<64, 128, 2>(a, st);
      else if (p.TN == 64 && p.TK == 256) launch_ring<64, 256, 2>(a, st);
      else if (p.TN == 128 && p.TK == 64) launch_ring<128, 64, 2>(a, st);
      else if (p.TN == 256 && p.TK == 64) launch_ring<256, 64, 2>(a, st);
      else launch_ring<128, 128, 2>(a, st);
      break;
    case kTwoBuf:
      if (d->c == 4) launch_2buf_tile<true>(p, a, st); else launch_2buf_tile<false>(p, a, st);
      break;
  }
  TOK_CHECK_LAUNCH("tok_conv_wgrad");
  if (dbias != nullptr && !cs_inline) {
    if (int e = tok_colsum_f32(a.cs, p.splitM, k_real, dbias, bias_accumulate, stream)) return e;
  }
  if (direct) return TOK_OK;
  if (flat) {
    if (tok_dbg_skip(2)) return TOK_OK;
    const size_t slab = (size_t)d->k * d->r * d->s * d->c;
    const size_t nb = (slab / 4 + 15) / 16;
    hipLaunchKernelGGL(wgrad_reduce_flat_kernel, dim3((int)(nb < 4096 ? nb : 4096)), dim3(256), 0, st,
                       (const float*)ws, dw, p.splitM, slab, accumulate, cs_inline ? a.ws_stride : slab,
                       cs_inline ? dbias : (float*)nullptr, k_real, cs_inline ? cs_pad : 0, bias_accumulate);
    TOK_CHECK_LAUNCH("tok_conv_wgrad(reduce)");
    return TOK_OK;
  }
  const size_t total = (size_t)k_real * d->r * d->s * c_real;
  const int blocks = (int)((total + 255) / 256 < 2048 ? (total + 255) / 256 : 2048);
  hipLaunchKernelGGL(wgrad_reduce_kernel, dim3(blocks), dim3(256), 0, st, (const float*)ws, dw,
                     p.splitM, k_real, d->r, d->s, c_real, d->k, d->s_pad, d->c, accumulate);
  TOK_CHECK_LAUNCH("tok_conv_wgrad(reduce)");
  return TOK_OK;
}
}
```

### torchok_amd/csrc/conv_win_epilogue.inc

```
#if TOK_WIN_EPI_PART == 1
  float s1r = 0.f, s2r = 0.f;
  float s1q = 0.f, s2q = 0.f;
  constexpr bool PST = WBN <= 64;
  float ps1[16], ps2[16];
  if constexpr (PST) {
#pragma unroll
    for (int c = 0; c < 16; ++c) { ps1[c] = 0.f; ps2[c] = 0.f; }
  }
#define TOK_S1(i) (PST ? ps1[(i) & 15] : s1[i])
#define TOK_S2(i) (PST ? ps2[(i) & 15] : s2[i])
#elif TOK_WIN_EPI_PART == 2
  auto epilogue = [&]() {
    const int nb = n0 + wn * WCH + sl * 8;
    if (a.bias != nullptr) {
#pragma unroll
      for (int c = 0; c < NH * 8; ++c) {
        const int n = nb + (c >> 3) * 32 + (c & 7);
        const float bv = n < a.K ? a.bias[n] : 0.f;
#pragma unroll
        for (int mt = 0; mt < MT; ++mt) acc[c >> 2][mt][c & 3] += bv;
      }
      if constexpr (QT) {
#pragma unroll
        for (int c = 0; c < 4; ++c) {
          const int n = n0 + NH * 32 + sl * 4 + c;
          const float bv = n < a.K ? a.bias[n] : 0.f;
#pragma unroll
          for (int mt = 0; mt < MT; ++mt) acc[2 * NH][mt][c] += bv;
        }
      }
    }
    const bool want_old = a.accumulate != 0;
    const bool want_y = a.stats != nullptr && !a.mask_store && a.bn_y != nullptr;
    const bool want_bits = a.bn_mask != nullptr && (a.mask_store || want_y);
    constexpr int SN = NH == 3 ? 32 : 16;
    float s1[SN], s2[SN];
    if constexpr (!PST) {
#pragma unroll
      for (int c = 0; c < SN; ++c) { s1[c] = 0.f; s2[c] = 0.f; }
    }
    constexpr int GQ = NH == 3 ? 1 : 2;
#pragma unroll
    for (int g = 0; g < MT; g += GQ) {
      bf16x8 pre_old[GQ][NH], pre_y[GQ][NH];
      unsigned pre_bits[GQ][NH];
      size_t pix[GQ];
      bool pok[GQ];
#pragma unroll
      for (int q = 0; q < GQ; ++q) {
        const int mt = g + q;
        const int gy = gyC + wm * WROWS_PER_WAVE + mt / SEGS, gx = gxC + (mt % SEGS) * 16 + li;
        pok[q] = gy < geo.BH && gx < a.W;
        pix[q] = TOK_WIN_PIXEL(gy, gx);
#pragma unroll
        for (int half = 0; half < NH; ++half) {
          const bool ok = pok[q] && nb + half * 32 + 8 <= a.K;
          const size_t eoff = pix[q] * a.K + nb + half * 32;
          pre_old[q][half] = (ok && want_old) ? ldg16(a.y + eoff) : zero8();
          pre_y[q][half] = (ok && want_y) ? ldg16(a.bn_y + eoff) : zero8();
          pre_bits[q][half] = (ok && want_bits) ? (unsigned)a.bn_mask[eoff >> 3] : 0xffu;
        }
      }
#pragma unroll
      for (int q = 0; q < GQ; ++q) {
        const int mt = g + q;
        if (!pok[q]) continue;
        bf16* yp = a.y + pix[q] * a.K + nb;
#pragma unroll
        for (int half = 0; half < NH; ++half) {
          if (nb + half * 32 + 8 > a.K) continue;
          float v[8];
#pragma unroll
          for (int e = 0; e < 8; ++e) v[e] = acc[half * 2 + (e >> 2)][mt][e & 3];
          if (a.accumulate) {
#pragma unroll
            for (int e = 0; e < 8; ++e) v[e] += bf2f(pre_old[q][half][e]);
          }
          bf16x8 o;
#pragma unroll
          for (int e = 0; e < 8; ++e) o[e] = f2bf(v[e]);
          if (a.mask_store) {
            const unsigned bits = pre_bits[q][half];
#pragma unroll
            for (int e = 0; e < 8; ++e) {
              if (!((bits >> e) & 1u)) o[e] = (bf16)0.f;
              TOK_S1(half * 8 + e) += bf2f(o[e]);
            }
          }
          stg16(yp + half * 32, o);
          if (a.stats != nullptr && !a.mask_store) {
            if (a.bn_y != nullptr) {
              const unsigned bits = pre_bits[q][half];
#pragma unroll
              for (int e = 0; e < 8; ++e) {
                const float dz = ((bits >> e) & 1u) ? bf2f(o[e]) : 0.f;
                TOK_S1(half * 8 + e) += dz;
                TOK_S2(half * 8 + e) = fmaf(dz, bf2f(pre_y[q][half][e]), TOK_S2(half * 8 + e));
              }
            } else {
#pragma unroll
              for (int e = 0; e < 8; ++e) {
                const float r = bf2f(o[e]);
                TOK_S1(half * 8 + e) += r;
                TOK_S2(half * 8 + e) = fmaf(r, r, TOK_S2(half * 8 + e));
              }
            }
          }
        }
        if constexpr (QT) {
          const int nq = n0 + NH * 32 + sl * 4;
          if (nq + 4 <= a.K) {
            const size_t eo = pix[q] * a.K + nq;
            float v[4];
#pragma unroll
            for (int e = 0; e < 4; ++e) v[e] = acc[2 * NH][mt][e];
            if (a.accumulate) {
              const bf16x4 old = *reinterpret_cast<const bf16x4*>(a.y + eo);
#pragma unroll
              for (int e = 0; e < 4; ++e) v[e] += bf2f(old[e]);
            }
            bf16x4 o;
#pragma unroll
            for (int e = 0; e < 4; ++e) o[e] = f2bf(v[e]);
            const unsigned bits = want_bits ? ((unsigned)a.bn_mask[eo >> 3] >> (unsigned)(eo & 4)) & 0xfu : 0xfu;
            if (a.mask_store) {
#pragma unroll
              for (int e = 0; e < 4; ++e) {
                if (!((bits >> e) & 1u)) o[e] = (bf16)0.f;
                TOK_S1(NH * 8 + e) += bf2f(o[e]);
              }
            }
            *reinterpret_cast<bf16x4*>(a.y + eo) = o;
            if (a.stats != nullptr && !a.mask_store) {
              if (a.bn_y != nullptr) {
                const bf16x4 yv = *reinterpret_cast<const bf16x4*>(a.bn_y + eo);
#pragma unroll
                for (int e = 0; e < 4; ++e) {
                  const float dz = ((bits >> e) & 1u) ? bf2f(o[e]) : 0.f;
                  TOK_S1(NH * 8 + e) += dz;
                  TOK_S2(NH * 8 + e) = fmaf(dz, bf2f(yv[e]), TOK_S2(NH * 8 + e));
                }
              } else {
#pragma unroll
                for (int e = 0; e < 4; ++e) {
                  const float r = bf2f(o[e]);
                  TOK_S1(NH * 8 + e) += r;
                  TOK_S2(NH * 8 + e) = fmaf(r, r, TOK_S2(NH * 8 + e));
                }
              }
            }
          }
        }
      }
    }
    if (!PST && a.stats != nullptr) {
#pragma unroll
      for (int base = 0; base < (NH == 3 ? 32 : 16); base += 16) {
#pragma unroll
        for (int step = 0; step < 4; ++step) {
          const int off = 8 >> step;
          const int cnt = 8 >> step;
          const bool up = (li & off) != 0;
#pragma unroll
          for (int j = 0; j < cnt; ++j) {
            const float send1 = up ? TOK_S1(base + j) : TOK_S1(base + j + cnt);
            const float send2 = up ? TOK_S2(base + j) : TOK_S2(base + j + cnt);
            const float keep1 = up ? TOK_S1(base + j + cnt) : TOK_S1(base + j);
            const float keep2 = up ? TOK_S2(base + j + cnt) : TOK_S2(base + j);
            TOK_S1(base + j) = keep1 + __shfl_xor(send1, off, 64);
            TOK_S2(base + j) = keep2 + __shfl_xor(send2, off, 64);
          }
        }
      }
      s1r += TOK_S1(0);
      s2r += TOK_S2(0);
      if constexpr (NH == 3) { s1q += TOK_S1(16); s2q += TOK_S2(16); }
    }
  };
#elif TOK_WIN_EPI_PART == 3
#undef TOK_S1
#undef TOK_S2
  if (PST && a.stats != nullptr) {
#pragma unroll
    for (int step = 0; step < 4; ++step) {
      const int off = 8 >> step;
      const int cnt = 8 >> step;
      const bool up = (li & off) != 0;
#pragma unroll
      for (int j = 0; j < cnt; ++j) {
        const float send1 = up ? ps1[j] : ps1[j + cnt];
        const float send2 = up ? ps2[j] : ps2[j + cnt];
        const float keep1 = up ? ps1[j + cnt] : ps1[j];
        const float keep2 = up ? ps2[j + cnt] : ps2[j];
        ps1[j] = keep1 + __shfl_xor(send1, off, 64);
        ps2[j] = keep2 + __shfl_xor(send2, off, 64);
      }
    }
    s1r = ps1[0];
    s2r = ps2[0];
  }
  if (a.stats != nullptr) {
    __syncthreads();
    float* red = reinterpret_cast<float*>(smem);
    const int nl = QT ? (li < 8 ? sl * 8 + li : 32 + sl * 4 + (li & 3)) : wn * WCH + (li >> 3) * 32 + sl * 8 + (li & 7);
    if (!QT || li < 12) {
      red[(0 * WGM + wm) * WBN + nl] = s1r;
      red[(1 * WGM + wm) * WBN + nl] = s2r;
    }
    if (NH == 3 && li < 8) {
      red[(0 * WGM + wm) * WBN + nl + 64] = s1q;
      red[(1 * WGM + wm) * WBN + nl + 64] = s2q;
    }
// ... 16 lines not shown
```

### torchok_amd/csrc/gemm256.hip

```cpp
#include "conv_common.h"
#include <stdlib.h>

namespace {

typedef __attribute__((address_space(3))) void lds_void;
typedef __attribute__((address_space(3))) char lds_char;

constexpr int GT = 256;
constexpr int GK = 64;
constexpr int TILE_B = GT * GK * 2;
constexpr int STAGE_B = 2 * TILE_B;
constexpr int NBLK = STAGE_B / 1024;
constexpr int NI = NBLK / 8;

__device__ __forceinline__ u32x4 lds_read16(uint32_t addr) {
  u32x4 v;
  asm volatile("ds_read_b128 %0, %1" : "=v"(v) : "v"(addr));
  return v;
}
__device__ __forceinline__ float row16_sum_f(float v) {
  v += __builtin_bit_cast(float, __builtin_amdgcn_update_dpp(0, __builtin_bit_cast(int, v), 0x128, 0xF, 0xF, false));
  v += __builtin_bit_cast(float, __builtin_amdgcn_update_dpp(0, __builtin_bit_cast(int, v), 0x124, 0xF, 0xF, false));
  v += __builtin_bit_cast(float, __builtin_amdgcn_update_dpp(0, __builtin_bit_cast(int, v), 0x122, 0xF, 0xF, false));
  v += __builtin_bit_cast(float, __builtin_amdgcn_update_dpp(0, __builtin_bit_cast(int, v), 0x121, 0xF, 0xF, false));
// ... 30 lines not shown
    n0 = nt * GT;
#pragma unroll
    for (int j = 0; j < NI; ++j) {
      const int bid = j * 8 + wave;
      const int row = (bid & 31) * 8 + (lane >> 3);
      const bool isw = bid < 32;
      const int grow = (isw ? n0 : m0) + row;
      const bool ok = grow < (isw ? a.K : a.M);
      voff[j] = ok ? (uint32_t)(((long long)grow * KD + kq[j]) * 2) : 0xFFFFFFF0u;
    }
  };
  auto issue = [&](int kt, int buf, bool live) {
#pragma unroll
    for (int j = 0; j < NI; ++j) {
      const int bid = j * 8 + wave;
      uint32_t off = (live && voff[j] != 0xFFFFFFF0u && kt * GK + kq[j] < KD) ? voff[j] + (uint32_t)(kt * (GK * 2)) : 0xFFFFFFF0u;
      asm volatile("" : "+v"(off));
      lds_void* dst = (lds_void*)(smem + buf * STAGE_B + bid * 1024);
      if (bid < 32) __builtin_amdgcn_raw_ptr_buffer_load_lds(wsrd, dst, 16, off, 0, 0, 0);
      else __builtin_amdgcn_raw_ptr_buffer_load_lds(xsrd, dst, 16, off, 0, 0, 0);
    }
  };

  const uint32_t swz = (uint32_t)((r & 3) | (((r >> 2) & 1) << 2));
  const uint32_t swx = (uint32_t)((r & 3) | (((r >> 3) & 1) << 2));
  const uint32_t a_lane = (uint32_t)((wn * 128 + 8 * (r >> 2) + (r & 3)) * 128);
  const uint32_t b_lane = (uint32_t)(TILE_B + (wm * 64 + r) * 128);
  uint32_t a_ch[2], b_ch[2];
#pragma unroll
  for (int kk = 0; kk < 2; ++kk) {
    a_ch[kk] = (((uint32_t)(4 * kk + g)) ^ swz) << 4;
    b_ch[kk] = (((uint32_t)(4 * kk + g)) ^ swx) << 4;
  }

  int tile = tok_xcd_remap(blockIdx.x, gridDim.x);
  int m0, n0;
  setup(tile, m0, n0);
  int base = 0;
  issue(0, base, tile < ntiles);
  while (tile < ntiles) {
  f32x4 acc[4][2][4];
#pragma unroll
  for (int p = 0; p < 4; ++p)
#pragma unroll
    for (int b = 0; b < 2; ++b)
#pragma unroll
      for (int mb = 0; mb < 4; ++mb) acc[p][b][mb] = (f32x4){0.f, 0.f, 0.f, 0.f};
  for (int kt = 0; kt < KT; ++kt) {
    const int buf = (base + kt) & 1;
    asm volatile("s_waitcnt vmcnt(0)" ::: "memory");
    __builtin_amdgcn_s_barrier();
    issue(kt + 1, buf ^ 1, kt + 1 < KT);
    const uint32_t sb = lds_base + (uint32_t)(buf * STAGE_B);
#pragma unroll
    for (int kk = 0; kk < 2; ++kk) {
      u32x4 af[4][2], bfr[4];
#pragma unroll
      for (int mb = 0; mb < 4; ++mb) bfr[mb] = lds_read16(sb + b_lane + (uint32_t)(mb * 16 * 128) + b_ch[kk]);
#pragma unroll
      for (int p = 0; p < 4; ++p)
#pragma unroll
        for (int b = 0; b < 2; ++b) af[p][b] = lds_read16(sb + a_lane + (uint32_t)((32 * p + 4 * b) * 128) + a_ch[kk]);
      asm volatile("s_waitcnt lgkmcnt(0)" ::: "memory");
      __builtin_amdgcn_sched_barrier(0);
#pragma unroll
      for (int p = 0; p < 4; ++p)
#pragma unroll
        for (int b = 0; b < 2; ++b)
#pragma unroll
          for (int mb = 0; mb < 4; ++mb)
            acc[p][b][mb] = __builtin_amdgcn_mfma_f32_16x16x32_bf16(__builtin_bit_cast(bf16x8, af[p][b]),
                                                                    __builtin_bit_cast(bf16x8, bfr[mb]), acc[p][b][mb], 0, 0, 0);
    }
  }
  const int cm0 = m0, cn0 = n0, cmt = m0 / GT;
  const int next = tile + gridDim.x;
  base = (base + KT) & 1;
  if (next < ntiles) {
    setup(next, m0, n0);
    issue(0, base, true);
  }

  float s1[4][8], s2[4][8];
  if constexpr (MODE >= 1 && MODE <= 3) {
#pragma unroll
    for (int p = 0; p < 4; ++p)
#pragma unroll
      for (int e = 0; e < 8; ++e) { s1[p][e] = 0.f; s2[p][e] = 0.f; }
  }
#pragma unroll
  for (int p = 0; p < 4; ++p) {
    const int n8 = cn0 + wn * 128 + 32 * p + 8 * g;
    const bool nok = n8 + 8 <= a.K;
    float bv[8];
#pragma unroll
    for (int e = 0; e < 8; ++e) bv[e] = (a.bias != nullptr && nok) ? a.bias[n8 + e] : 0.f;
#pragma unroll
    for (int mb = 0; mb < 4; ++mb) {
      const int pix = cm0 + wm * 64 + 16 * mb + r;
      if (pix < a.M && nok) {
        const size_t off = (size_t)pix * a.K + n8;
        float v[8];
#pragma unroll
        for (int e = 0; e < 8; ++e) v[e] = acc[p][e >> 2][mb][e & 3] + bv[e];
        if (a.accumulate) {
          const bf16x8 old = ldg16(a.y + off);
#pragma unroll
          for (int e = 0; e < 8; ++e) v[e] += bf2f(old[e]);
        }
        bf16x8 o;
#pragma unroll
        for (int e = 0; e < 8; ++e) o[e] = f2bf(v[e]);
        if constexpr (MODE == 3) {
          const unsigned bits = (unsigned)a.bn_mask[off >> 3];
#pragma unroll
          for (int e = 0; e < 8; ++e) {
            if (!((bits >> e) & 1u)) o[e] = (bf16)0.f;
            s1[p][e] += bf2f(o[e]);
          }
        }
        stg16(a.y + off, o);
        if constexpr (MODE == 1) {
#pragma unroll
          for (int e = 0; e < 8; ++e) {
            const float q = bf2f(o[e]);
            s1[p][e] += q;
            s2[p][e] = fmaf(q, q, s2[p][e]);
          }
        }
        if constexpr (MODE == 2) {
          const bf16x8 yv = ldg16(a.bn_y + off);
          const unsigned bits = a.bn_mask != nullptr ? (unsigned)a.bn_mask[off >> 3] : 0xffu;
#pragma unroll
          for (int e = 0; e < 8; ++e) {
            const float dz = ((bits >> e) & 1u) ? bf2f(o[e]) : 0.f;
            s1[p][e] += dz;
            s2[p][e] = fmaf(dz, bf2f(yv[e]), s2[p][e]);
          }
        }
      }
    }
  }
  if constexpr (MODE >= 1 && MODE <= 3) {
    float* red = reinterpret_cast<float*>(smem + 2 * STAGE_B);
#pragma unroll
    for (int p = 0; p < 4; ++p)
#pragma unroll
      for (int e = 0; e < 8; ++e) {
        const float t1 = row16_sum_f(s1[p][e]), t2 = row16_sum_f(s2[p][e]);
        if (r == 15) {
          const int nl = wn * 128 + 32 * p + 8 * g + e;
          red[(0 * 4 + wm) * GT + nl] = t1;
          red[(1 * 4 + wm) * GT + nl] = t2;
        }
      }
    asm volatile("s_waitcnt lgkmcnt(0)" ::: "memory");
    __builtin_amdgcn_s_barrier();
    const int which = tid >> 8, c = tid & 255;
    const float t = red[(which * 4 + 0) * GT + c] + red[(which * 4 + 1) * GT + c] + red[(which * 4 + 2) * GT + c] +
                    red[(which * 4 + 3) * GT + c];
    const int n = cn0 + c;
    if (n < a.K) a.stats[((size_t)which * a.stat_rows + cmt) * a.K + n] = t;
    if (cmt == a.gridM - 1 && n < a.K)
      for (int rr = a.gridM; rr < a.stat_rows; ++rr) a.stats[((size_t)which * a.stat_rows + rr) * a.K + n] = 0.f;
    asm volatile("s_waitcnt lgkmcnt(0)" ::: "memory");
    __builtin_amdgcn_s_barrier();
  }
  tile = next;
  }
  asm volatile("s_waitcnt vmcnt(0) lgkmcnt(0)" ::: "memory");
}

int g256_flag() {
  static const int v = [] { const char* e = getenv("TOK_GEMM256"); return (int)(e ? atoi(e) : 1); }();
  return v;
}
int g256_min_k() {
  static const int v = [] { const char* e = getenv("TOK_GEMM256_MIN_K"); return (int)(e ? atoi(e) : 256); }();
  return v;
}
int g256_min_tiles() {
  static const int v = [] { const char* e = getenv("TOK_GEMM256_MIN_TILES"); return (int)(e ? atoi(e) : 128); }();
  return v;
}

}

bool gemm256_modes(const ConvArgs& a) {
  if (a.ep_scale != nullptr || a.sub != nullptr) return false;
  if (a.mask_store && (a.bn_mask == nullptr || a.stats == nullptr)) return false;
  if (a.y2 != nullptr || a.act_x != nullptr) return false;
  return true;
}
bool gemm256_serves(const ConvArgs& a) { return gemm256_geometry(a) && gemm256_modes(a); }

bool gemm256_geometry(const ConvArgs& a) {
  const int flag = g256_flag();
  if (!flag) return false;
  if (!(a.R == 1 && a.S == 1 && a.stride == 1 && a.pad == 0 && a.C != 4)) return false;
  if (a.Ktot % 8 != 0 || a.K % 8 != 0 || a.Ktot <= GK) return false;
  if (flag >= 3) return true;
  if (a.K < 192 || a.M < 4096) return false;
  const long long tiles = (long long)tok_cdiv(a.M, GT) * tok_cdiv(a.K, GT);
  const int nt = tok_cdiv(a.K, GT);
  if ((long long)nt * GT * 3 > (long long)a.K * 4) return false;
  if (tiles < g256_min_tiles()) return false;
  if (flag >= 2) return a.Ktot >= g256_min_k();
  return a.Ktot >= 384;
}

int gemm256_rows(const ConvArgs& a) { return (tok_cdiv(a.M, GT) + 7) / 8 * 8; }

void gemm256_tiles(const ConvArgs& a, int* gridM, int* gridN) { *gridM = tok_cdiv(a.M, GT); *gridN = tok_cdiv(a.K, GT); }
int gemm256_grid(int gridM, int gridN) { return gridM * gridN < 256 ? gridM * gridN : 256; }

int gemm256_launch(ConvArgs& a, hipStream_t st) {
  constexpr int smem = 2 * STAGE_B + 2 * 4 * GT * 4;
  const int grid = a.grid;
  if (a.mask_store) tok_launch_lds<&gemm256_kernel<3>>(smem, dim3(grid), dim3(512), smem, st, a);
  else if (a.stats == nullptr) tok_launch_lds<&gemm256_kernel<0>>(smem, dim3(grid), dim3(512), smem, st, a);
  else if (a.bn_y == nullptr) tok_launch_lds<&gemm256_kernel<1>>(smem, dim3(grid), dim3(512), smem, st, a);
  else tok_launch_lds<&gemm256_kernel<2>>(smem, dim3(grid), dim3(512), smem, st, a);
  return 0;
}
```

### torchok_amd/csrc/pw_gemm.hip

```cpp
#include "pw_gemm.h"
#include <stdlib.h>

namespace {

constexpr int BK = 64;
constexpr int BM = 128;

__device__ __forceinline__ int fw_swz(int n) {
  return ((0x78 >> (((n >> 3) & 3) << 1)) & 3) | (((n >> 1) & 1) << 2);
}

struct PwDiv { uint32_t mul, shift; };
PwDiv make_pwdiv(uint32_t d) {
  PwDiv f = {0, 0};
  if (d <= 1) return f;
  uint32_t l = 0;
  while ((1ull << l) < d) ++l;
  f.mul = (uint32_t)((((1ull << 32) * ((1ull << l) - d)) / d) + 1);
  f.shift = l;
  return f;
}
__device__ __forceinline__ uint32_t pwdiv(uint32_t n, PwDiv f) { return (uint32_t)(((uint64_t)__umulhi(n, f.mul) + n) >> f.shift); }

__device__ __forceinline__ u32x4 lds_read16(uint32_t addr) {
// ... 202 lines not shown
#pragma unroll
    for (int t = 0; t < 4; ++t)
#pragma unroll
      for (int mt = 0; mt < MT; ++mt)
        acc[t][mt] = __builtin_amdgcn_mfma_f32_16x16x32_bf16(__builtin_bit_cast(bf16x8, wf[1][t]), __builtin_bit_cast(bf16x8, af[1][mt]),
                                                             acc[t][mt], 0, 0, 0);
  };

  auto etile = [&](uint32_t sb, bf16x8 (&dst)[MT][2]) {
    u32x4 raw[MT][2];
#pragma unroll
    for (int mt = 0; mt < MT; ++mt)
#pragma unroll
      for (int half = 0; half < 2; ++half)
        raw[mt][half] = lds_read16(sb + wn * A_BYTES + (arow0 + mt * 16) * 128 + (((sl + 4 * half) ^ aswz) << 4));
    asm volatile("s_waitcnt lgkmcnt(0)" ::: "memory");
    __builtin_amdgcn_sched_barrier(0);
#pragma unroll
    for (int mt = 0; mt < MT; ++mt)
#pragma unroll
      for (int half = 0; half < 2; ++half) dst[mt][half] = __builtin_bit_cast(bf16x8, raw[mt][half]);
  };

  auto add_e1 = [&](uint32_t sb) {
    bf16x8 ev[MT][2];
    etile(sb, ev);
#pragma unroll
    for (int mt = 0; mt < MT; ++mt)
#pragma unroll
      for (int half = 0; half < 2; ++half)
#pragma unroll
        for (int e = 0; e < 8; ++e) acc[half * 2 + (e >> 2)][mt][e & 3] += bf2f(ev[mt][half][e]);
  };

  auto epilogue = [&](int it, uint32_t sb) {
    const int m0 = it * BM;
    const int nb = n0 + wn * 64 + sl * 8;
    bf16x8 ev[MT][2];
    const bool need_tile = BNEP ? (a.e1 != nullptr) : (a.e2 != nullptr);
    if (need_tile) etile(sb, ev);
    uint32_t mbits[MT][2];
    if (a.mask_in != nullptr) {
#pragma unroll
      for (int mt = 0; mt < MT; ++mt)
#pragma unroll
        for (int half = 0; half < 2; ++half)
          mbits[mt][half] = lds_read_u8(sb + A_BYTES + W_BYTES + (arow0 + mt * 16) * (BN / 8) + wn * 8 + sl + half * 4);
      asm volatile("s_waitcnt lgkmcnt(0)" ::: "memory");
      __builtin_amdgcn_sched_barrier(0);
    }
#pragma unroll
    for (int mt = 0; mt < MT; ++mt) {
      const int m = m0 + arow0 + mt * 16;
      if (m >= a.M) continue;
      bf16* yp = a.y + (size_t)m * a.N + nb;
#pragma unroll
      for (int half = 0; half < 2; ++half) {
        if (nb + half * 32 + 8 > a.N) continue;
        float v[8];
#pragma unroll
        for (int e = 0; e < 8; ++e) v[e] = acc[half * 2 + (e >> 2)][mt][e & 3] + bia[half * 8 + e];
        bf16x8 o;
#pragma unroll
        for (int e = 0; e < 8; ++e) o[e] = f2bf(v[e]);
        const size_t eoff = (size_t)m * a.N + nb + half * 32;
        if (BNEP) {
          unsigned bits = 0;
#pragma unroll
          for (int e = 0; e < 8; ++e) {
            float z = fmaf(v[e], esc[half * 8 + e], esh[half * 8 + e]);
            if (a.e1 != nullptr) z += bf2f(ev[mt][half][e]);
            if (a.ep_relu) z = fmaxf(z, 0.f);
            o[e] = f2bf(z);
            bits |= (bf2f(o[e]) > 0.f ? 1u : 0u) << e;
          }
          if (a.mask_out != nullptr) a.mask_out[eoff >> 3] = (uint8_t)bits;
        }
        if (a.mask_store) {
          const unsigned bits = mbits[mt][half];
#pragma unroll
          for (int e = 0; e < 8; ++e) {
            if (!((bits >> e) & 1u)) o[e] = (bf16)0.f;
            s1[half * 8 + e] += bf2f(o[e]);
          }
        }
        stg16(yp + half * 32, o);
        if (a.stats != nullptr && !a.mask_store) {
          if (a.e2 != nullptr) {
            const unsigned bits = a.mask_in != nullptr ? mbits[mt][half] : 0xffu;
#pragma unroll
            for (int e = 0; e < 8; ++e) {
              const float dz = ((bits >> e) & 1u) ? bf2f(o[e]) : 0.f;
              s1[half * 8 + e] += dz;
              s2[half * 8 + e] = fmaf(dz, bf2f(ev[mt][half][e]), s2[half * 8 + e]);
            }
          } else {
#pragma unroll
            for (int e = 0; e < 8; ++e) {
              const float r = bf2f(o[e]);
              s1[half * 8 + e] += r;
              s2[half * 8 + e] = fmaf(r, r, s2[half * 8 + e]);
            }
          }
        }
      }
    }
  };

  zero_acc();
  issue(0);
  issue(1);
  int cur = 0, nxt = 2;
  int itC = it0, ksC = 0;
  for (int s = 0; s < total; ++s) {
    asm volatile("s_waitcnt vmcnt(%0) lgkmcnt(0)" ::"n"(LOADS) : "memory");
    __builtin_amdgcn_s_barrier();
    issue(nxt);
    const uint32_t sb = lds_base + cur * STAGE;
    if (ksC < KT) {
      compute(sb);
    } else if (!BNEP && a.accumulate && ksC == KT) {
      add_e1(sb);
    }
    if (ksC == SPT - 1) {
      epilogue(itC, sb);
      zero_acc();
      ksC = 0;
      itC += sweep;
    } else {
      ++ksC;
    }
    cur = cur == NST - 1 ? 0 : cur + 1;
    nxt = nxt == NST - 1 ? 0 : nxt + 1;
  }
  asm volatile("s_waitcnt vmcnt(0) lgkmcnt(0)" ::: "memory");

  if (a.stats != nullptr) {
    __syncthreads();
    float* red = reinterpret_cast<float*>(smem);
#pragma unroll
    for (int step = 0; step < 4; ++step) {
      const int off = 8 >> step;
      const int cnt = 8 >> step;
      const bool up = (li & off) != 0;
#pragma unroll
      for (int j = 0; j < cnt; ++j) {
        const float send1 = up ? s1[j] : s1[j + cnt];
        const float send2 = up ? s2[j] : s2[j + cnt];
        const float keep1 = up ? s1[j + cnt] : s1[j];
        const float keep2 = up ? s2[j + cnt] : s2[j];
        s1[j] = keep1 + __shfl_xor(send1, off, 64);
        s2[j] = keep2 + __shfl_xor(send2, off, 64);
      }
    }
    const int nl = wn * 64 + (li >> 3) * 32 + sl * 8 + (li & 7);
    red[(0 * WGM + wm) * BN + nl] = s1[0];
    red[(1 * WGM + wm) * BN + nl] = s2[0];
    __syncthreads();
    if (tid < 2 * BN) {
      const int which = tid / BN;
      const int c = tid - which * BN;
      float t = 0.f;
#pragma unroll
      for (int w_ = 0; w_ < WGM; ++w_) t += red[(which * WGM + w_) * BN + c];
      const int row = xcd * S8 + jm;
      const int n = n0 + c;
// ... 56 lines not shown
```

### torchok_amd/engine/functional.py

```python
import weakref
from typing import Optional, Tuple

import os

import torch
from torch import nn

from .. import _C
from .core import _ms as _core_ms
from . import paramgrad as PG
from .core import BF16, Node, Region, TTensor, await_ready, donate_grad, grad_target, is_last_contribution, pad8, ptr, stream_ptr

F32 = torch.float32



class _Packs:
    __slots__ = ('fwd', 'dgrad', 'bias', 'key', 'synced', 'dims')

    def __init__(self):
        self.fwd = None
        self.dgrad = None
        self.bias = None
        self.key = None
# ... 148 lines not shown
    q = (w + 2 * pad - s) // stride + 1
    return _C.ConvDesc(n, h, w, cp, k_pad, r, s, p, q, stride, pad, 8 if cp == 4 else s)


def _check_conv(conv: nn.Conv2d):
    if conv.groups != 1 or tuple(conv.dilation) != (1, 1):
        raise NotImplementedError('torchok_amd conv: dilation == 1 and groups == 1 (dense, conv_bn_act), groups == channels '
                                  '(depthwise 3x3 / 5x5, dwconv_bn_act) or a grouped 3x3 of group width 4, 8, 16, 32 or 64 '
                                  '(gconv_bn_act) only')
    if conv.kernel_size[0] != conv.kernel_size[1] or conv.stride[0] != conv.stride[1] \
            or conv.padding[0] != conv.padding[1] or isinstance(conv.padding, str):
        raise NotImplementedError('torchok_amd conv: square kernel / stride / padding only')
    if conv.padding_mode != 'zeros':
        raise NotImplementedError('torchok_amd conv: zero padding only')



RELU = 'relu'
HARD_SWISH = 'hard_swish'
RELU6 = 'relu6'
MASKLESS = {HARD_SWISH: 'hswish', RELU6: 'relu6'}


def _check_act(relu, act, bn, shortcut=None, pool=False, defer_apply=False):
    if act is None:
        return RELU if relu else None
    if act not in MASKLESS:
        raise NotImplementedError(f'torchok_amd activation {act!r}: None (ReLU / identity by `relu`), {HARD_SWISH!r} or {RELU6!r}')
    if bn is None or shortcut is not None or pool or defer_apply:
        raise NotImplementedError(f"act={act!r}: BatchNorm units without shortcut, pool or defer_apply only")
    return act


def _maskless(lib, act, stage):
    name = f'tok_bn_{MASKLESS[act]}_{stage}'
    return getattr(lib, name), name



def batch_stats(bn: nn.BatchNorm2d) -> bool:
    return bn.training or bn.running_mean is None


def bn_coeffs(lib, st, bn, stats, rows, m, kp, dev):
    vec = torch.empty((4, kp), dtype=F32, device=dev)
    scale, shift = vec[0], vec[1]
    if stats is None:
        _C.check(lib.tok_bn_eval_coeffs(ptr(bn.weight), ptr(bn.bias), ptr(bn.running_mean), ptr(bn.running_var),
                                        float(bn.eps), kp, bn.num_features, ptr(scale), ptr(shift), st), 'tok_bn_eval_coeffs')
        return scale, shift, None, None
    if bn.momentum is None:
        raise NotImplementedError('BatchNorm momentum=None (cumulative average)')
    mean, rstd = vec[2], vec[3]
    track = bn.training and bn.track_running_stats and bn.running_mean is not None
    _C.check(lib.tok_bn_finalize(ptr(stats), rows, m, kp, bn.num_features, ptr(bn.weight), ptr(bn.bias),
                                 ptr(bn.running_mean) if track else None, ptr(bn.running_var) if track else None,
                                 ptr(bn.num_batches_tracked) if track else None, float(bn.momentum), float(bn.eps),
                                 ptr(mean), ptr(rstd), ptr(scale), ptr(shift), st), 'tok_bn_finalize')
    return scale, shift, mean, rstd


def bn_apply(lib, st, y, scale, shift, act, shortcut, want_mask, m, kp):
    out_data = torch.empty_like(y)
    if act in MASKLESS:
        fwd, name = _maskless(lib, act, 'fwd')
        _C.check(fwd(ptr(y), ptr(scale), ptr(shift), ptr(out_data), m, kp, st), name)
        return out_data, None
    mask = torch.empty((m, kp // 8), dtype=torch.uint8, device=y.device) if want_mask else None
    _C.check(lib.tok_bn_act_fwd(ptr(y), ptr(scale), ptr(shift), ptr(shortcut.data) if shortcut is not None else None,
                                int(act == RELU), ptr(out_data), ptr(mask), m, kp, st), 'tok_bn_act_fwd')
    return out_data, mask


class _ConvBnActNode(Node):
    needs_backward = True
    act = None
    relu = property(lambda self: self.act == RELU)

    def __init__(self):
        self.x = self.out = self.shortcut = None
        self.y = self.mask = None
        self.region = None
        self.fused_partial = None
        self.pool = None
        self.ypool = None

    def release(self):
        self.x = self.out = self.shortcut = None
        self.y = self.pk = self.mask = self.fused_partial = self.pool = self.ypool = None
        self.mean = self.rstd = self.scale = self.shift = None

    def wants_fused_bwd_stats(self) -> bool:
        return (self.bn is not None and self.batch_stats and self.pool is None
                and (self.act is None or (self.act == RELU and self.mask is not None)))

    def _apply_bwd(self, lib, st, g, mask, coef, dy, ds_ptr, ds_acc, m, kp):
        if self.act in MASKLESS:
            bwd_apply, name = _maskless(lib, self.act, 'bwd_apply')
            _C.check(bwd_apply(ptr(g), ptr(self.y), ptr(self.scale), ptr(self.shift), ptr(coef), ptr(dy), m, kp, st), name)
        else:
            _C.check(lib.tok_bn_bwd_apply(ptr(g), ptr(self.y), ptr(mask), ptr(self.scale), ptr(self.shift), ptr(coef),
                                          int(self.relu), ptr(dy), ds_ptr, ds_acc, m, kp, st), 'tok_bn_bwd_apply')

    def _finalize_bwd(self, lib, st, g, mask, m, kp, g_need, b_need):
        bn = self.bn
        dzy = 0
        if self.fused_partial is not None:
            partial, rows = self.fused_partial
            dzy = 1
        else:
            rows = lib.tok_bn_bwd_rows(m, kp)
            if self.pool is not None and self.ypool is not None:
                mp = self.out.data.numel() // kp
                rows = lib.tok_bn_bwd_rows(mp, kp)
                partial = torch.empty((2, rows, kp), dtype=F32, device=g.device)
                _C.check(lib.tok_bn_pool_bwd_reduce_pooled(ptr(g), ptr(self.out.data), ptr(self.ypool), ptr(self.mean),
                                                           ptr(self.rstd), mp, kp, ptr(partial), st),
                         'tok_bn_pool_bwd_reduce_pooled')
            elif self.pool is not None:
                partial = torch.empty((2, rows, kp), dtype=F32, device=g.device)
                n_, h_, w_, _ = self.y.shape
                _C.check(lib.tok_bn_pool_bwd_reduce(ptr(g), ptr(self.pool), ptr(self.y), ptr(self.scale), ptr(self.shift),
                                                    ptr(self.mean), ptr(self.rstd), n_, h_, w_, kp, ptr(partial), st),
                         'tok_bn_pool_bwd_reduce')
            elif self.act in MASKLESS:
                partial = torch.empty((2, rows, kp), dtype=F32, device=g.device)
                bwd_reduce, name = _maskless(lib, self.act, 'bwd_reduce')
                _C.check(bwd_reduce(ptr(g), ptr(self.y), ptr(self.scale), ptr(self.shift), ptr(self.mean), ptr(self.rstd), m, kp,
                                    ptr(partial), st), name)
            else:
                partial = torch.empty((2, rows, kp), dtype=F32, device=g.device)
                _C.check(lib.tok_bn_bwd_reduce(ptr(g), ptr(self.y), ptr(mask), ptr(self.scale), ptr(self.shift),
                                               ptr(self.mean), ptr(self.rstd), int(self.relu), m, kp, ptr(partial), st),
                         'tok_bn_bwd_reduce')
        coef = torch.empty((3, kp), dtype=F32, device=g.device)
        gbuf, bbuf, acc, finish = PG.pair_sinks(bn.weight if g_need else None, bn.bias if b_need else None)
        _C.check(lib.tok_bn_bwd_finalize(ptr(partial), rows, m, kp, bn.num_features, ptr(bn.weight), ptr(self.mean),
                                         ptr(self.rstd), ptr(gbuf), ptr(bbuf), ptr(coef), acc, dzy, st), 'tok_bn_bwd_finalize')
        finish()
        return coef

    def _bn_bwd(self, lib, st, g, m, kp, need_dy, apply=None):
        bn = self.bn
        g_need, b_need = bn.weight.requires_grad, bn.bias.requires_grad
        mask = self.mask if self.act == RELU else None
        if self.batch_stats:
            coef = self._finalize_bwd(lib, st, g, mask, m, kp, g_need, b_need)
        else:
            if g_need or b_need:
                raise NotImplementedError('gradients of BatchNorm affine parameters in eval mode')
            coef = torch.zeros((3, kp), dtype=F32, device=g.device)
            coef[0] = self.scale
        if not need_dy:
            return None
        dy = torch.empty_like(self.y)
        if apply is not None:
            apply(mask, coef, dy)
        else:
            self._apply_bwd(lib, st, g, mask, coef, dy, None, 0, m, kp)
        return dy

    def backward(self):
        lib, st = _C.lib(), stream_ptr()
        out: TTensor = self.out
        g = out.grad
        if g is None:
            return
        apply_event = None
        conv, bn, d = self.conv, self.bn, self.desc
        m, kp = self.y.numel() // self.y.shape[-1], self.y.shape[-1]
        x: TTensor = self.x
        w_need = conv.weight.requires_grad
        x_need = x.requires_grad
        bias_need = conv.bias is not None and conv.bias.requires_grad
        sc: Optional[TTensor] = self.shortcut
        side = w_need and PG.goes_side(self, g, PG.CONV, m)

        if bn is not None:
            sc_need = sc is not None and sc.requires_grad

            def apply(mask, coef, dy):
                nonlocal apply_event
                if side and self.pool is None and self.act not in MASKLESS:
                    apply_event = self.region.raw_event()
                ds_ptr, ds_acc = None, 0
                if sc_need:
                    if sc.grad is None and out.grad_owned:
                        ds_ptr = ptr(g)
                        donate_grad(sc, g)
                    else:
                        tgt, ds_acc = grad_target(sc)
                        ds_ptr = ptr(tgt)
                if self.pool is not None:
                    n_, h_, w_, _ = self.y.shape
                    _C.check(lib.tok_bn_pool_bwd_apply(ptr(g), ptr(self.pool), ptr(self.y), ptr(self.scale), ptr(self.shift),
                                                       ptr(coef), n_, h_, w_, kp, ptr(dy), st), 'tok_bn_pool_bwd_apply')
                    return
                if apply_event is not None:
                    lib.tok_next_launch_event(apply_event)
                try:
                    self._apply_bwd(lib, st, g, mask, coef, dy, ds_ptr, ds_acc, m, kp)
                finally:
                    if apply_event is not None:
                        lib.tok_next_launch_event(None)
            dy = self._bn_bwd(lib, st, g, m, kp, w_need or x_need or bias_need or sc_need, apply)
        else:
            dy = g
        out.grad = None
        if dy is None:
            return
        bias_in_wgrad = bool(bias_need and w_need and PG.wgrad_plan(d)[0])
        if bias_need and not bias_in_wgrad:
            bs, bacc = PG.sink(conv.bias)
            PG.colsum(dy, m, kp, bs, bacc, two_pass=m > 4096 and kp == conv.bias.shape[0], n_real=conv.bias.shape[0])
            PG.commit(conv.bias, bs, bacc)
        if w_need:
            k, _, _, c = _krsc(conv.weight)
            PG.run_beside(self, side, (x.data, dy), raw_event=apply_event, fn=lambda: PG.weight_grad(
                d, x.data, dy, k, c, weight=conv.weight, bias=conv.bias if bias_in_wgrad else None)[1:])
        if x_need:
            prod = x.node
            rider = _dgrad_rider(x)
            sub = x.grad_sub if getattr(self, 'sub_capable', False) else None
            tgt, acc = grad_target(x, sub_ok=sub is not None)
            partial = _rider_partial(lib, rider, prod, d, x.cp, g.device)
            bn_y = ptr(prod.y) if rider == BN_SUMS else None
            bn_mask = ptr(prod.mask) if (rider == MASKED_DZ or (rider == BN_SUMS and prod.relu)) else None
            if sub is not None:
                x.grad_sub = None
                assert acc == 0
                _C.check(lib.tok_conv_dgrad_subacc(d, ptr(dy), ptr(self.pk.dgrad), ptr(tgt), ptr(sub), bn_y, bn_mask, ptr(partial),
                                                   int(rider == MASKED_DZ), st), 'tok_conv_dgrad_subacc')
            elif rider == MASKED_DZ:
                _C.check(lib.tok_conv_dgrad_maskstore(d, ptr(dy), ptr(self.pk.dgrad), ptr(tgt), acc, bn_mask, ptr(partial), st),
                         'tok_conv_dgrad_maskstore')
            elif rider == BN_SUMS:
                _C.check(lib.tok_conv_dgrad_bnstats(d, ptr(dy), ptr(self.pk.dgrad), ptr(tgt), acc, bn_y, bn_mask, ptr(partial), st),
                         'tok_conv_dgrad_bnstats')
            else:
                _C.check(lib.tok_conv_dgrad(d, ptr(dy), ptr(self.pk.dgrad), ptr(tgt), acc, st), 'tok_conv_dgrad')


BN_SUMS = 'bn_sums'
MASKED_DZ = 'masked_dz'


def _dgrad_rider(x: TTensor):
    prod = x.node
    if (isinstance(prod, _ConvBnActNode) and is_last_contribution(x) and prod.wants_fused_bwd_stats()
            and prod.fused_partial is None):
        return BN_SUMS
    if (isinstance(prod, _Unit3Node) and prod.relu and prod.mask is not None and is_last_contribution(x)
            and prod.masked_partial is None):
        return MASKED_DZ
    return None


def _rider_partial(lib, rider, prod, d, cp: int, dev) -> Optional[torch.Tensor]:
    if rider is None:
        return None
    rows = lib.tok_conv_dgrad_stat_rows(d)
    partial = torch.empty((2, rows, cp), dtype=F32, device=dev)
    if rider == MASKED_DZ:
        prod.masked_partial = (partial, rows)
    else:
        prod.fused_partial = (partial, rows)
    return partial



FUSE_UNIT3 = os.environ.get('TOK_FUSE_UNIT3', '1') != '0'
UNIT3_MIN_ROWS = int(os.environ.get('TOK_UNIT3_MIN_ROWS', '100000'))


def _pointwise_desc(x: TTensor, k: int) -> _C.ConvDesc:
    n, h, w, cp = x.shape
    return _C.ConvDesc(n, h, w, cp, k, 1, 1, h, w, 1, 0, 1)


def _colsum_f32(t: torch.Tensor, m: int, c: int) -> torch.Tensor:
    out = torch.empty(c, dtype=F32, device=t.device)
    PG.colsum(t, m, c, out, 0, two_pass=m > 4096, n_real=c)
    return out


class _Unit3Node(Node):
    needs_backward = True

    def __init__(self):
        self.x = self.out = self.shortcut = self.mask = None
        self.relu = True
        self.masked_partial = None

    def release(self):
        self.x = self.out = self.shortcut = self.mask = self.masked_partial = None
        self.mean = self.rstd = self.wz = self.zsum = self.pk = None

    def backward(self):
        lib, st = _C.lib(), stream_ptr()
        out: TTensor = self.out
        g = out.grad
        if g is None:
            return
        conv, bn, d, x, sc = self.conv, self.bn, self.desc, self.x, self.shortcut
        kp, p = d.k, d.c
        m = d.n * d.p * d.q
        dev = g.device
        if self.masked_partial is not None:
            partial, rows = self.masked_partial
            dz = g
        else:
            rows = lib.tok_bn_bwd_rows(m, kp)
            partial = torch.empty((2, rows, kp), dtype=F32, device=dev)
            dz = g if (out.grad_owned or not self.relu) else torch.empty_like(g)
            _C.check(lib.tok_relu_mask_reduce(ptr(g), ptr(self.mask) if self.relu else None, m, kp, ptr(dz), ptr(partial), st),
                     'tok_relu_mask_reduce')
        out.grad = None
        if sc is not None and sc.requires_grad:
            if donate_grad(sc, dz):
                scn = sc.node
                if isinstance(scn, _Unit3Node) and not scn.relu and sc.uses == 1 and scn.masked_partial is None:
                    scn.masked_partial = (partial, rows)
            else:
                tgt, _ = grad_target(sc)
                tgt.add_(dz)
        w_need = conv.weight.requires_grad
        x_need = x.requires_grad
        g_need, b_need = bn.weight.requires_grad, bn.bias.requires_grad
        if not (w_need or x_need or g_need or b_need):
            return
        G = PG.weight_grad(d, x.data, dz, kp, p)[0]
        gbuf, bbuf, pacc, finish = PG.pair_sinks(bn.weight if g_need else None, bn.bias if b_need else None)
        dw, wacc = PG.sink(conv.weight) if w_need else (torch.empty((kp, p), dtype=F32, device=dev), 0)
        coef = torch.empty((3, kp), dtype=F32, device=dev)
        wa = torch.empty((p, kp), dtype=BF16, device=dev)
        wb = torch.empty((p, p), dtype=BF16, device=dev)
        cvec = torch.empty(p, dtype=F32, device=dev)
        scratch = torch.empty(lib.tok_bn3_bwd_prepare_ws_floats(p, kp), dtype=F32, device=dev)
        _C.check(lib.tok_bn3_bwd_prepare(ptr(G), ptr(conv.weight), ptr(self.wz), ptr(self.zsum), ptr(partial), rows, m, p,
                                         kp, ptr(bn.weight), ptr(self.mean), ptr(self.rstd), ptr(gbuf), ptr(bbuf), pacc,
                                         ptr(coef), ptr(dw), wacc, ptr(wa), ptr(wb), ptr(cvec), ptr(scratch), st),
                 'tok_bn3_bwd_prepare')
        finish()
        if w_need:
            PG.commit(conv.weight, dw, wacc)
        if not x_need:
            return
        prod = x.node
        fuse = _dgrad_rider(x) == BN_SUMS
        tgt, acc = grad_target(x)
        dpp = _pointwise_desc(x, p)
        part2 = _rider_partial(lib, BN_SUMS if fuse else None, prod, dpp, p, dev)
        bn_y = ptr(prod.y) if fuse else None
        bn_mask = ptr(prod.mask) if (fuse and prod.relu) else None
        if lib.tok_conv_dgrad2_ok(d, dpp):
            _C.check(lib.tok_conv_dgrad2(d, ptr(dz), ptr(wa), dpp, ptr(x.data), ptr(wb), ptr(cvec), ptr(tgt), acc, bn_y, bn_mask,
                                         ptr(part2), st), 'tok_conv_dgrad2')
        else:
            _C.check(lib.tok_conv_dgrad(d, ptr(dz), ptr(wa), ptr(tgt), acc, st), 'tok_conv_dgrad')
            _C.check(lib.tok_conv_dgrad_bias(dpp, ptr(x.data), ptr(wb), ptr(cvec), ptr(tgt), 1, bn_y, bn_mask, ptr(part2), st),
                     'tok_conv_dgrad_bias')
        if self.region is not None:
            self.region.keep_until_join(dz, wa, wb, cvec, G, scratch)


def _unit3_forward(region: Region, x: TTensor, conv: nn.Conv2d, bn: nn.BatchNorm2d, shortcut: Optional[TTensor], kp: int,
                   relu: bool) -> TTensor:
    lib, st = _C.lib(), stream_ptr()
    dev = x.data.device
    if bn.momentum is None:
        raise NotImplementedError('BatchNorm momentum=None (cumulative average)')
    d = _pointwise_desc(x, kp)
    p = x.cp
    m = d.n * d.p * d.q
    pk = get_packs(conv.weight, None, kp, 1, p, want_dgrad=False, refresh=True)
    dz_ = _pointwise_desc(x, p)
    zz = PG.weight_grad(dz_, x.data, x.data, p, p)[0]
    if x.colsum_part is not None:
        part, nrows = x.colsum_part
        zsum = torch.empty(p, dtype=F32, device=x.data.device)
        _C.check(lib.tok_colsum_f32(ptr(part), nrows, p, ptr(zsum), 0, st), 'tok_colsum_f32')
        x.colsum_part = None
    else:
        zsum = _colsum_f32(x.data, m, p)
    mean, rstd, scale, shift = (torch.empty(kp, dtype=F32, device=dev) for _ in range(4))
    wz = torch.empty((kp, p), dtype=F32, device=dev)
    track = bn.training and bn.track_running_stats and bn.running_mean is not None
    _C.check(lib.tok_bn_gram_finalize(ptr(zz), ptr(zsum), ptr(conv.weight), m, p, kp, ptr(bn.weight), ptr(bn.bias),
                                      ptr(bn.running_mean) if track else None, ptr(bn.running_var) if track else None,
                                      ptr(bn.num_batches_tracked) if track else None, float(bn.momentum), float(bn.eps),
                                      ptr(mean), ptr(rstd), ptr(scale), ptr(shift), ptr(wz), st), 'tok_bn_gram_finalize')
    out_data = torch.empty((d.n, d.p, d.q, kp), dtype=BF16, device=dev)
    training = region.grad_mode and (conv.weight.requires_grad or x.requires_grad or bn.weight.requires_grad
                                     or (shortcut is not None and shortcut.requires_grad))
    mask = torch.empty((m, kp // 8), dtype=torch.uint8, device=dev) if (training and relu) else None
    _C.check(lib.tok_conv_fwd_bn_apply(d, ptr(x.data), ptr(pk.fwd), ptr(scale), ptr(shift),
                                       ptr(shortcut.data) if shortcut is not None else None, int(relu), ptr(out_data),
                                       ptr(mask), st), 'tok_conv_fwd_bn_apply')
    out = TTensor(out_data, kp, requires_grad=bool(training))
    if training:
        node = _Unit3Node()
        node.x, node.out, node.shortcut, node.mask, node.relu = x, out, shortcut, mask, relu
        node.conv, node.bn, node.desc, node.pk = conv, bn, d, pk
        node.mean, node.rstd, node.wz, node.zsum = mean, rstd, wz, zsum
        out.node = node
        if x.requires_grad:
            x.uses += 1
        if shortcut is not None and shortcut.requires_grad:
            shortcut.uses += 1
        region.add(node)
    return out


FUSE_STEM_POOL = os.environ.get('TOK_FUSE_STEM_POOL', '1') != '0'
# ... 596 lines not shown
```

### torchok_amd/engine/paramgrad.py

```python
import torch

from .. import _C
from . import core
from .core import grad_slot, ptr, stream_ptr

F32 = torch.float32


def sink(p: torch.nn.Parameter):
    slot = grad_slot(p)
    g = p.grad
    return slot, int(g is not None and g.data_ptr() == slot.data_ptr())


def commit(p: torch.nn.Parameter, slot: torch.Tensor, accumulate: int):
    if not accumulate:
        if p.grad is None:
            p.grad = slot
        else:
            p.grad.add_(slot)
    for h in core.param_grad_hooks:
        h(p)


def store(dst: torch.Tensor, accumulate: int, value: torch.Tensor):
    if accumulate:
        dst.add_(value)
    else:
        dst.copy_(value)


def pair_sinks(p0, p1):
    s0 = sink(p0) if p0 is not None else None
    s1 = sink(p1) if p1 is not None else None
    if s0 is not None and s1 is not None and s0[1] != s1[1]:
        t0, t1 = torch.empty_like(s0[0]), torch.empty_like(s1[0])

        def finish():
            store(s0[0], s0[1], t0)
            commit(p0, *s0)
            store(s1[0], s1[1], t1)
            commit(p1, *s1)
        return t0, t1, 0, finish

    def finish():
        if s0 is not None:
            commit(p0, *s0)
        if s1 is not None:
            commit(p1, *s1)
    one = s0 if s0 is not None else s1
    return (s0[0] if s0 is not None else None, s1[0] if s1 is not None else None, one[1] if one is not None else 0, finish)


_plans = {}


def wgrad_plan(d: _C.ConvDesc):
    lib = _C.lib()
    key = (bytes(d), id(lib))
    p = _plans.get(key)
    if p is None:
        p = _plans[key] = (bool(lib.tok_conv_wgrad_bias_ok(d)), int(lib.tok_conv_wgrad_bias_ws_bytes(d)),
                           int(lib.tok_conv_wgrad_ws_bytes(d)))
    return p


def weight_grad(d: _C.ConvDesc, x: torch.Tensor, dy: torch.Tensor, k: int, c: int, weight=None, out=None, accumulate=0,
                bias=None, bias_out=None):
    lib = _C.lib()
    rides = bias is not None or bias_out is not None
    ws_bytes = wgrad_plan(d)[1 if rides else 2]
    ws = torch.empty(max(ws_bytes // 4, 1), dtype=F32, device=x.device)
    if weight is not None:
        dst, acc = sink(weight)
    else:
        dst, acc = out if out is not None else torch.empty((k, c), dtype=F32, device=x.device), accumulate
    if rides:
        bdst, bacc = sink(bias) if bias is not None else (bias_out, 0)
        _C.check(lib.tok_conv_wgrad_bias(d, ptr(x), ptr(dy), ptr(dst), k, c, ptr(ws), ws_bytes, acc, ptr(bdst), bacc,
                                         stream_ptr()), 'tok_conv_wgrad_bias')
        if bias is not None:
            commit(bias, bdst, bacc)
    else:
        _C.check(lib.tok_conv_wgrad(d, ptr(x), ptr(dy), ptr(dst), k, c, ptr(ws), ws_bytes, acc, stream_ptr()),
                 'tok_conv_wgrad')
    if weight is not None:
        commit(weight, dst, acc)
    return dst, ws


def colsum(dy: torch.Tensor, m: int, n_pad: int, dst: torch.Tensor, accumulate: int, two_pass: bool, n_real: int = 0):
    lib, st = _C.lib(), stream_ptr()
    if not two_pass:
        _C.check(lib.tok_colsum(ptr(dy), m, n_pad, n_real, ptr(dst), accumulate, st), 'tok_colsum')
        return None
    nrows = lib.tok_colsum_partial_rows(m, n_pad)
    part = torch.empty((nrows, n_pad), dtype=F32, device=dy.device)
    _C.check(lib.tok_colsum_partial(ptr(dy), m, n_pad, ptr(part), st), 'tok_colsum_partial')
    _C.check(lib.tok_colsum_f32(ptr(part), nrows, n_pad, ptr(dst), accumulate, st), 'tok_colsum_f32')
    return part


CONV = 'conv'
TOKEN = 'token'
NECK = 'neck'


def goes_side(node, g: torch.Tensor, policy: str, rows: int = 0) -> bool:
    from . import functional as EF
    if not (EF.WGRAD_SIDE_STREAM and g.is_cuda and node.region is not None):
        return False
    if policy != TOKEN and not EF._side_for_tag(node.stream_tag, node.region):
        return False
    if policy == CONV:
        w = node.conv.weight
        r, s = (w.shape[2], w.shape[3]) if w.dim() == 4 else (1, 1)
        if not EF._wgrad_side_ok(r, s, rows, w.shape[0], w.shape[1]):
            return False
    return not torch.cuda.is_current_stream_capturing()


def run_beside(node, side: bool, reads, fn, raw_event=None):
    if not side:
        fn()
        return
    with node.region.fork_side(reads, raw_event=raw_event):
        node.region.keep_until_join(*(fn() or ()))
```

Measured before the change: 14440.

## Fuse paired 1x1 weight-gradient GEMMs and store masked dz with BN stats in dgrad

Adds a two-input wgrad ring kernel that computes the Gram/weight gradients of a bottleneck's main 1x1 conv and its projection shortcut in one launch, sharing the same dy stream. The second unit reuses the precomputed gram instead of launching its own wgrad. Separately, a new dgrad 'maskstats' epilogue writes the relu-masked dz and accumulates both BN sums (including the dz*y product) in one pass. This lets the later BN backward apply skip re-masking and reuse the stored gradient. The cost is extra epilogue register pressure, a larger workspace and more complex routing.

```diff
diff --git a/include/tok.h b/include/tok.h
--- a/include/tok.h
+++ b/include/tok.h
@@ -87,6 +87,10 @@
 int tok_conv_dgrad_subacc(const tok_conv_desc* d, const void* dy, const void* w_dgrad, void* dx, const void* dsub,
                           const void* bn_y , const uint8_t* mask ,
                           float* partial , int mask_store, void* stream);
+int tok_conv_dgrad_maskstats_ok(const tok_conv_desc* d, int with_sub);
+int tok_conv_dgrad_maskstats(const tok_conv_desc* d, const void* dy, const void* w_dgrad, void* dx, int accumulate,
+                             const void* dsub , const void* bn_y, const uint8_t* mask, float* partial,
+                             void* stream);
 int tok_conv_dgrad2_ok(const tok_conv_desc* d1, const tok_conv_desc* d2);
 int tok_conv_dgrad2(const tok_conv_desc* d1, const void* dy1, const void* w1_dgrad, const tok_conv_desc* d2, const void* dy2,
                     const void* w2_dgrad, const float* bias , void* dx, int accumulate,
@@ -96,6 +100,10 @@
 int tok_conv_wgrad(const tok_conv_desc* d, const void* x, const void* dy, float* dw,
                    int k_real, int c_real, void* ws, size_t ws_bytes, int accumulate,
                    void* stream);
+int tok_conv_wgrad2_ok(const tok_conv_desc* d1, const tok_conv_desc* d2);
+size_t tok_conv_wgrad2_ws_bytes(const tok_conv_desc* d1, const tok_conv_desc* d2);
+int tok_conv_wgrad2(const tok_conv_desc* d1, const void* x1, const tok_conv_desc* d2, const void* x2, const void* dy,
+                    float* dw1, int accumulate1, float* dw2, int accumulate2, void* ws, size_t ws_bytes, void* stream);
 int tok_conv_wgrad_bias_ok(const tok_conv_desc* d);
 size_t tok_conv_wgrad_bias_ws_bytes(const tok_conv_desc* d);
 int tok_conv_wgrad_bias(const tok_conv_desc* d, const void* x, const void* dy, float* dw, int k_real, int c_real,
diff --git a/torchok_amd/_C.py b/torchok_amd/_C.py
--- a/torchok_amd/_C.py
+++ b/torchok_amd/_C.py
@@ -93,6 +93,11 @@
     'tok_subsample2_bwd': (c_int, [_P, c_int, c_int, c_int, c_int, _P, c_int, _P]),
     'tok_conv_dgrad_subacc_ok': (c_int, [POINTER(ConvDesc)]),
     'tok_conv_dgrad_subacc': (c_int, [POINTER(ConvDesc), _P, _P, _P, _P, _P, _P, _P, c_int, _P]),
+    'tok_conv_wgrad2_ok': (c_int, [POINTER(ConvDesc), POINTER(ConvDesc)]),
+    'tok_conv_wgrad2_ws_bytes': (c_size_t, [POINTER(ConvDesc), POINTER(ConvDesc)]),
+    'tok_conv_wgrad2': (c_int, [POINTER(ConvDesc), _P, POINTER(ConvDesc), _P, _P, _P, c_int, _P, c_int, _P, c_size_t, _P]),
+    'tok_conv_dgrad_maskstats_ok': (c_int, [POINTER(ConvDesc), c_int]),
+    'tok_conv_dgrad_maskstats': (c_int, [POINTER(ConvDesc), _P, _P, _P, c_int, _P, _P, _P, _P, _P]),
     'tok_softmax_ce_fwd': (c_int, [_P, _P, c_int, c_int, c_int, c_int64, _P, _P, _P, _P]),
     'tok_softmax_ce_bwd': (c_int, [_P, _P, _P, _P, _P, c_int, c_int, c_int, c_int64, _P, _P]),
     'tok_softmax_ce_smooth_fwd': (c_int, [_P, _P, c_int, c_int, c_int, c_int64, c_float, _P, _P, _P, _P]),
diff --git a/torchok_amd/csrc/conv_igemm.hip b/torchok_amd/csrc/conv_igemm.hip
--- a/torchok_amd/csrc/conv_igemm.hip
+++ b/torchok_amd/csrc/conv_igemm.hip
@@ -374,7 +374,7 @@
     bf16x8 pre_old[MT][2], pre_y[MT][2];
     unsigned pre_bits[MT][2];
     const bool want_old = a.accumulate != 0;
-    const bool want_y = a.stats != nullptr && !a.mask_store && a.bn_y != nullptr;
+    const bool want_y = a.stats != nullptr && a.bn_y != nullptr;
     const bool want_bits = a.bn_mask != nullptr && (a.mask_store || want_y);
     constexpr bool PRE = !BNEP && !ACT && !C4;
     if (PRE) {
@@ -453,6 +453,11 @@
               for (int e = 0; e < 8; ++e) {
                 if (!((bits >> e) & 1u)) o[e] = (bf16)0.f;
                 s1[half * 8 + e] += bf2f(o[e]);
+              }
+              if (a.bn_y != nullptr) {
+                const bf16x8 yv = PRE ? pre_y[mt][half] : ldg16(a.bn_y + opix * a.K + nb + half * 32);
+#pragma unroll
+                for (int e = 0; e < 8; ++e) s2[half * 8 + e] = fmaf(bf2f(o[e]), bf2f(yv[e]), s2[half * 8 + e]);
               }
             }
             if (NTS) __builtin_nontemporal_store(o, reinterpret_cast<bf16x8*>(yp + half * 32));
@@ -987,6 +992,25 @@
 }
 
 
+extern "C" int tok_conv_dgrad_maskstats_ok(const tok_conv_desc* d, int with_sub) {
+  if (check_desc(d, "tok_conv_dgrad_maskstats_ok")) return 0;
+  ConvArgs a = {};
+  if (dgrad_fill(d, a)) return 0;
+  if (!with_sub) return 1;
+  return (d->c % 64 == 0 && tok_conv_dgrad_subacc_ok(d)) ? 1 : 0;
+}
+
+extern "C" int tok_conv_dgrad_maskstats(const tok_conv_desc* d, const void* dy, const void* w_dgrad, void* dx, int accumulate,
+                                        const void* dsub, const void* bn_y, const uint8_t* mask, float* partial, void* stream) {
+  TOK_CHECK_ARG(bn_y && mask && partial, "tok_conv_dgrad_maskstats: bn_y / mask / partial must not be null");
+  TOK_CHECK_ARG(dsub == nullptr || !accumulate, "tok_conv_dgrad_maskstats: dsub is the accumulated operand (accumulate must be 0)");
+  TOK_CHECK_ARG(dsub == nullptr || (d != nullptr && d->c % 64 == 0), "tok_conv_dgrad_maskstats: dsub needs c a multiple of 64");
+  DgradEpilogue ep = {}; ep.accumulate = accumulate; ep.bn_y = bn_y; ep.bn_mask = mask; ep.partial = partial; ep.mask_store = 1;
+  ep.sub = dsub;
+  return dgrad_impl(d, dy, w_dgrad, dx, ep, stream, "tok_conv_dgrad_maskstats");
+}
+
+
 namespace {
 bool dgrad2_route(const tok_conv_desc* d1, const tok_conv_desc* d2, ConvRoute* r) {
   if (d1 == nullptr || d2 == nullptr) return false;
diff --git a/torchok_amd/csrc/conv_wgrad.hip b/torchok_amd/csrc/conv_wgrad.hip
--- a/torchok_amd/csrc/conv_wgrad.hip
+++ b/torchok_amd/csrc/conv_wgrad.hip
@@ -18,6 +18,11 @@
   int cs_cols;
   int adv_q, adv_p;
   size_t cs_stride, ws_stride;
+  const bf16* x2;
+  float* ws2;
+  int C2, tilesK1;
+  uint32_t x2_bytes;
+  size_t ws2_stride;
 };
 
 __device__ __forceinline__ uint32_t magic_div(uint32_t n, uint32_t mul, uint32_t shift) {
@@ -271,7 +276,7 @@
 }
 
 
-template <int TN, int TK, int WK>
+template <int TN, int TK, int WK, bool TWO = false>
 __global__ __launch_bounds__(128 * WK, WK == 4 ? 1 : 0) void conv_wgrad_ring_kernel(WgradArgs a) {
   constexpr int MS = 32, NST = 3, NTHR = 128 * WK;
   constexpr int CN = TN / 8, CK = TK / 8;
@@ -298,6 +303,9 @@
   const int t = id - split * ntile;
   const int tn = t / a.tilesK;
   const int tk = t - tn * a.tilesK;
+  const bool second = TWO && tk >= a.tilesK1;
+  const int tkl = second ? tk - a.tilesK1 : tk;
+  const int Cx = second ? a.C2 : a.C;
 
   const int mstart = split * a.mchunk;
   const int mend = min(a.M, mstart + a.mchunk);
@@ -313,15 +321,15 @@
 
   int kc0;
   bool k_ok;
-  if constexpr (WK == 2) {
+  if constexpr (WK == 2 && !TWO) {
     const int k0 = tk * TK + xlog * 8;
     const int tap = k0 / a.C;
     kc0 = k0 - tap * a.C;
     const int kr = tap / a.S;
     k_ok = kr < a.R;
   } else {
-    kc0 = tk * TK + xlog * 8;
-    k_ok = kc0 < a.C;
+    kc0 = tkl * TK + xlog * 8;
+    k_ok = kc0 < Cx;
   }
 
   int xm[XP];
@@ -330,7 +338,8 @@
   int ym = mstart + yrow;
 
   const __amdgpu_buffer_rsrc_t ysrd = __builtin_amdgcn_make_buffer_rsrc((void*)a.dy, 0, a.dy_bytes, 0x00020000);
-  const __amdgpu_buffer_rsrc_t xsrd = __builtin_amdgcn_make_buffer_rsrc((void*)a.x, 0, a.x_bytes, 0x00020000);
+  const __amdgpu_buffer_rsrc_t xsrd =
+      __builtin_amdgcn_make_buffer_rsrc((void*)(second ? a.x2 : a.x), 0, second ? a.x2_bytes : a.x_bytes, 0x00020000);
   typedef __attribute__((address_space(3))) void lds_void;
 
   auto issue = [&](int dbuf) {
@@ -346,7 +355,7 @@
     ym += MS;
 #pragma unroll
     for (int i = 0; i < XP; ++i) {
-      uint32_t off = (k_ok && xm[i] < mend) ? (uint32_t)(xm[i] * a.C + kc0) * 2u : 0xFFFFFFF0u;
+      uint32_t off = (k_ok && xm[i] < mend) ? (uint32_t)(xm[i] * Cx + kc0) * 2u : 0xFFFFFFF0u;
       asm volatile("" : "+v"(off));
       __builtin_amdgcn_raw_ptr_buffer_load_lds(xsrd, (lds_void*)(Xdst + i * RPX * XS), 16, off, 0, 0, 0);
       xm[i] += MS;
@@ -456,16 +465,17 @@
       }
   }
 
-  float* out = a.ws + (size_t)split * a.ws_stride;
+  float* out = second ? a.ws2 + (size_t)split * a.ws2_stride : a.ws + (size_t)split * a.ws_stride;
+  const int Kt = TWO ? Cx : a.Ktot;
 #pragma unroll
   for (int i = 0; i < NT; ++i) {
 #pragma unroll
     for (int j = 0; j < KTL; ++j) {
-      const int kcol = tk * TK + wk * (TK / WK) + j * 16 + li;
+      const int kcol = tkl * TK + wk * (TK / WK) + j * 16 + li;
 #pragma unroll
       for (int r = 0; r < 4; ++r) {
         const int n = tn * TN + wn2 * (TN / 2) + i * 16 + g * 4 + r;
-        if (n < a.K && kcol < a.Ktot) out[(size_t)n * a.Ktot + kcol] = acc[i][j][r];
+        if (n < a.K && kcol < Kt) out[(size_t)n * Kt + kcol] = acc[i][j][r];
       }
     }
   }
@@ -956,6 +966,13 @@
   chunk = (chunk + MS - 1) / MS * MS;
   p.mchunk = (int)chunk;
   p.splitM = (int)((M + chunk - 1) / chunk);
+}
+
+static int ring_split_target(int TN, int TK, long long M) {
+  const int stage = 32 * (TN + TK) * 2;
+  const int per_cu = (160 * 1024) / (3 * stage);
+  static const int ring_target = tok_env_int("TOK_WGRAD_WGS", 0), long_target = tok_env_int("TOK_WGRAD_WGS_LONG", 0);
+  return (long_target > 0 && M >= 100000) ? long_target : ring_target > 0 ? ring_target : 256 * (per_cu > 2 ? 2 : per_cu);
 }
 
 Plan make_plan(const tok_conv_desc* d) {
@@ -990,12 +1007,7 @@
     }
     p.tilesN = tok_cdiv(d->k, p.TN);
     p.tilesK = tok_cdiv(Ktot, p.TK);
-    const int stage = 32 * (p.TN + p.TK) * 2;
-    const int per_cu = (160 * 1024) / (3 * stage);
-    static const int ring_target = tok_env_int("TOK_WGRAD_WGS", 0), long_target = tok_env_int("TOK_WGRAD_WGS_LONG", 0);
-    const int target = (long_target > 0 && M >= 100000) ? long_target
-                       : ring_target > 0 ? ring_target : 256 * (per_cu > 2 ? 2 : per_cu);
-    split_m(p, M, target, p.tilesN * p.tilesK, 32, 512);
+    split_m(p, M, ring_split_target(p.TN, p.TK, M), p.tilesN * p.tilesK, 32, 512);
     return p;
   }
   p.route = stem_wgrad_serves(d) ? kStem : kTwoBuf;
@@ -1010,10 +1022,10 @@
   return p;
 }
 
-template <int TN, int TK, int WK>
+template <int TN, int TK, int WK, bool TWO = false>
 void launch_ring(const WgradArgs& a, hipStream_t st) {
   constexpr int smem = 3 * 32 * (TN + TK) * 2;
-  tok_launch_lds<&conv_wgrad_ring_kernel<TN, TK, WK>>(smem, dim3(a.tilesN * a.tilesK * a.splitM), dim3(128 * WK), smem, st, a);
+  tok_launch_lds<&conv_wgrad_ring_kernel<TN, TK, WK, TWO>>(smem, dim3(a.tilesN * a.tilesK * a.splitM), dim3(128 * WK), smem, st, a);
 }
 
 template <int TN, int TK, bool C4, int MS>
@@ -1097,7 +1109,7 @@
   const bool flat = (k_real == d->k) && (c_real == d->c) && (d->s_pad == d->s) &&
                     (((size_t)d->k * d->r * d->s * d->c) % 4 == 0) && (((uintptr_t)dw & 15) == 0);
   const bool direct = flat && p.splitM == 1 && !accumulate;
-  WgradArgs a;
+  WgradArgs a = {};
   a.x = (const bf16*)x; a.dy = (const bf16*)dy; a.ws = direct ? dw : (float*)ws;
   a.H = d->h; a.W = d->w; a.C = d->c; a.K = d->k; a.R = d->r; a.S = d->s_pad; a.P = d->p; a.Q = d->q;
   a.stride = d->stride; a.pad = d->pad;
@@ -1173,3 +1185,83 @@
   return TOK_OK;
 }
 }
+
+
+namespace {
+struct Plan2 { int TN, TK, tilesN, tilesK1, tilesK2, splitM, mchunk; };
+
+bool make_plan2(const tok_conv_desc* d1, const tok_conv_desc* d2, Plan2& q) {
+  if (d1 == nullptr || d2 == nullptr) return false;
+  for (const tok_conv_desc* d : {d1, d2})
+    if (!(d->r == 1 && d->s == 1 && d->s_pad == 1 && d->stride == 1 && d->pad == 0 && d->c % 8 == 0 && d->k % 8 == 0 &&
+          d->n > 0 && d->h > 0 && d->w > 0 && d->p == d->h && d->q == d->w)) return false;
+  const long long M = (long long)d1->n * d1->p * d1->q;
+  if (d1->k != d2->k || d1->k < 128 || M != (long long)d2->n * d2->p * d2->q) return false;
+  if ((unsigned long long)M * d1->k * 2 >= 0xFFFFFFF0ull || (unsigned long long)M * d1->c * 2 >= 0xFFFFFFF0ull ||
+      (unsigned long long)M * d2->c * 2 >= 0xFFFFFFF0ull) return false;
+  q.TK = (d1->c <= 64 || d2->c <= 64) ? 64 : 128;
+  q.TN = q.TK == 64 && d1->k >= 256 ? 256 : 128;
+  q.tilesN = tok_cdiv(d1->k, q.TN);
+  q.tilesK1 = tok_cdiv(d1->c, q.TK);
+  q.tilesK2 = tok_cdiv(d2->c, q.TK);
+  const Plan p = make_plan(d1);
+  q.splitM = p.splitM; q.mchunk = p.mchunk;
+  return true;
+}
+}
+
+extern "C" int tok_conv_wgrad2_ok(const tok_conv_desc* d1, const tok_conv_desc* d2) {
+  Plan2 q;
+  return make_plan2(d1, d2, q) ? 1 : 0;
+}
+
+extern "C" size_t tok_conv_wgrad2_ws_bytes(const tok_conv_desc* d1, const tok_conv_desc* d2) {
+  Plan2 q;
+  if (!make_plan2(d1, d2, q)) return 0;
+  return (size_t)q.splitM * d1->k * ((size_t)d1->c + d2->c) * sizeof(float);
+}
+
+extern "C" int tok_conv_wgrad2(const tok_conv_desc* d1, const void* x1, const tok_conv_desc* d2, const void* x2, const void* dy,
+                               float* dw1, int accumulate1, float* dw2, int accumulate2, void* ws, size_t ws_bytes,
+                               void* stream) {
+  Plan2 q;
+  TOK_CHECK_ARG(make_plan2(d1, d2, q), "tok_conv_wgrad2: layers not served (ask tok_conv_wgrad2_ok)");
+  TOK_CHECK_ARG(x1 && x2 && dy && dw1 && dw2 && ws, "tok_conv_wgrad2: null pointer");
+  TOK_CHECK_ARG((((uintptr_t)dw1 | (uintptr_t)dw2 | (uintptr_t)ws) & 15) == 0, "tok_conv_wgrad2: dw1 / dw2 / ws must be 16-byte aligned");
+  const size_t need = tok_conv_wgrad2_ws_bytes(d1, d2);
+  if (ws_bytes < need) {
+    tok_set_error("tok_conv_wgrad2: workspace %zu < %zu bytes", ws_bytes, need);
+    return TOK_ERR_WORKSPACE;
+  }
+  if (tok_dbg_skip(16)) return TOK_OK;
+  const size_t slab1 = (size_t)d1->k * d1->c, slab2 = (size_t)d1->k * d2->c;
+  WgradArgs a = {};
+  a.x = (const bf16*)x1; a.x2 = (const bf16*)x2; a.dy = (const bf16*)dy;
+  a.ws = (float*)ws; a.ws2 = (float*)ws + (size_t)q.splitM * slab1;
+  a.ws_stride = slab1; a.ws2_stride = slab2;
+  a.H = d1->h; a.W = d1->w; a.C = d1->c; a.C2 = d2->c; a.K = d1->k; a.R = 1; a.S = 1; a.P = d1->p; a.Q = d1->q;
+  a.stride = 1; a.pad = 0;
+  a.M = d1->n * d1->p * d1->q; a.PQ = d1->p * d1->q; a.HW = d1->h * d1->w;
+  a.Ktot = d1->c;
+  a.tilesN = q.tilesN; a.tilesK1 = q.tilesK1; a.tilesK = q.tilesK1 + q.tilesK2; a.splitM = q.splitM; a.mchunk = q.mchunk;
+  a.x_bytes = (uint32_t)((unsigned long long)a.M * d1->c * 2);
+  a.x2_bytes = (uint32_t)((unsigned long long)a.M * d2->c * 2);
+  a.dy_bytes = (uint32_t)((unsigned long long)a.M * d1->k * 2);
+  hipStream_t st = tok_stream(stream);
+  if (q.TN == 256) launch_ring<256, 64, 2, true>(a, st);
+  else if (q.TK == 64) launch_ring<128, 64, 2, true>(a, st);
+  else launch_ring<128, 128, 2, true>(a, st);
+  TOK_CHECK_LAUNCH("tok_conv_wgrad2");
+  if (tok_dbg_skip(2)) return TOK_OK;
+  const float* wsrc[2] = {a.ws, a.ws2};
+  float* dst[2] = {dw1, dw2};
+  const size_t slab[2] = {slab1, slab2};
+  const int acc[2] = {accumulate1, accumulate2};
+  for (int i = 0; i < 2; ++i) {
+    const size_t nb = (slab[i] / 4 + 15) / 16;
+    hipLaunchKernelGGL(wgrad_reduce_flat_kernel, dim3((int)(nb < 4096 ? nb : 4096)), dim3(256), 0, st, wsrc[i], dst[i], q.splitM,
+                       slab[i], acc[i], slab[i], (float*)nullptr, 0, 0, 0);
+    TOK_CHECK_LAUNCH("tok_conv_wgrad2(reduce)");
+  }
+  return TOK_OK;
+}
diff --git a/torchok_amd/csrc/conv_win_epilogue.inc b/torchok_amd/csrc/conv_win_epilogue.inc
--- a/torchok_amd/csrc/conv_win_epilogue.inc
+++ b/torchok_amd/csrc/conv_win_epilogue.inc
@@ -31,7 +31,7 @@
       }
     }
     const bool want_old = a.accumulate != 0;
-    const bool want_y = a.stats != nullptr && !a.mask_store && a.bn_y != nullptr;
+    const bool want_y = a.stats != nullptr && a.bn_y != nullptr;
     const bool want_bits = a.bn_mask != nullptr && (a.mask_store || want_y);
     constexpr int SN = NH == 3 ? 32 : 16;
     float s1[SN], s2[SN];
@@ -86,6 +86,11 @@
               if (!((bits >> e) & 1u)) o[e] = (bf16)0.f;
               TOK_S1(half * 8 + e) += bf2f(o[e]);
             }
+            if (a.bn_y != nullptr) {
+#pragma unroll
+              for (int e = 0; e < 8; ++e)
+                TOK_S2(half * 8 + e) = fmaf(bf2f(o[e]), bf2f(pre_y[q][half][e]), TOK_S2(half * 8 + e));
+            }
           }
           stg16(yp + half * 32, o);
           if (a.stats != nullptr && !a.mask_store) {
@@ -128,6 +133,11 @@
               for (int e = 0; e < 4; ++e) {
                 if (!((bits >> e) & 1u)) o[e] = (bf16)0.f;
                 TOK_S1(NH * 8 + e) += bf2f(o[e]);
+              }
+              if (a.bn_y != nullptr) {
+                const bf16x4 yv = *reinterpret_cast<const bf16x4*>(a.bn_y + eo);
+#pragma unroll
+                for (int e = 0; e < 4; ++e) TOK_S2(NH * 8 + e) = fmaf(bf2f(o[e]), bf2f(yv[e]), TOK_S2(NH * 8 + e));
               }
             }
             *reinterpret_cast<bf16x4*>(a.y + eo) = o;
diff --git a/torchok_amd/csrc/gemm256.hip b/torchok_amd/csrc/gemm256.hip
--- a/torchok_amd/csrc/gemm256.hip
+++ b/torchok_amd/csrc/gemm256.hip
@@ -136,11 +136,23 @@
   }
 
   float s1[4][8], s2[4][8];
-  if constexpr (MODE >= 1 && MODE <= 3) {
+  if constexpr (MODE >= 1) {
 #pragma unroll
     for (int p = 0; p < 4; ++p)
 #pragma unroll
       for (int e = 0; e < 8; ++e) { s1[p][e] = 0.f; s2[p][e] = 0.f; }
+  }
+  unsigned mbits[4][4];
+  if constexpr (MODE == 4) {
+#pragma unroll
+    for (int p = 0; p < 4; ++p) {
+      const int n8 = cn0 + wn * 128 + 32 * p + 8 * g;
+#pragma unroll
+      for (int mb = 0; mb < 4; ++mb) {
+        const int pix = cm0 + wm * 64 + 16 * mb + r;
+        mbits[p][mb] = (pix < a.M && n8 + 8 <= a.K) ? (unsigned)a.bn_mask[((size_t)pix * a.K + n8) >> 3] : 0u;
+      }
+    }
   }
 #pragma unroll
   for (int p = 0; p < 4; ++p) {
@@ -165,13 +177,18 @@
         bf16x8 o;
 #pragma unroll
         for (int e = 0; e < 8; ++e) o[e] = f2bf(v[e]);
-        if constexpr (MODE == 3) {
-          const unsigned bits = (unsigned)a.bn_mask[off >> 3];
+        if constexpr (MODE == 3 || MODE == 4) {
+          const unsigned bits = MODE == 4 ? mbits[p][mb] : (unsigned)a.bn_mask[off >> 3];
 #pragma unroll
           for (int e = 0; e < 8; ++e) {
             if (!((bits >> e) & 1u)) o[e] = (bf16)0.f;
             s1[p][e] += bf2f(o[e]);
           }
+        }
+        if constexpr (MODE == 4) {
+          const bf16x8 yv = ldg16(a.bn_y + off);
+#pragma unroll
+          for (int e = 0; e < 8; ++e) s2[p][e] = fmaf(bf2f(o[e]), bf2f(yv[e]), s2[p][e]);
         }
         stg16(a.y + off, o);
         if constexpr (MODE == 1) {
@@ -195,7 +212,7 @@
       }
     }
   }
-  if constexpr (MODE >= 1 && MODE <= 3) {
+  if constexpr (MODE >= 1) {
     float* red = reinterpret_cast<float*>(smem + 2 * STAGE_B);
 #pragma unroll
     for (int p = 0; p < 4; ++p)
@@ -271,7 +288,8 @@
 int gemm256_launch(ConvArgs& a, hipStream_t st) {
   constexpr int smem = 2 * STAGE_B + 2 * 4 * GT * 4;
   const int grid = a.grid;
-  if (a.mask_store) tok_launch_lds<&gemm256_kernel<3>>(smem, dim3(grid), dim3(512), smem, st, a);
+  if (a.mask_store && a.bn_y != nullptr) tok_launch_lds<&gemm256_kernel<4>>(smem, dim3(grid), dim3(512), smem, st, a);
+  else if (a.mask_store) tok_launch_lds<&gemm256_kernel<3>>(smem, dim3(grid), dim3(512), smem, st, a);
   else if (a.stats == nullptr) tok_launch_lds<&gemm256_kernel<0>>(smem, dim3(grid), dim3(512), smem, st, a);
   else if (a.bn_y == nullptr) tok_launch_lds<&gemm256_kernel<1>>(smem, dim3(grid), dim3(512), smem, st, a);
   else tok_launch_lds<&gemm256_kernel<2>>(smem, dim3(grid), dim3(512), smem, st, a);
diff --git a/torchok_amd/csrc/pw_gemm.hip b/torchok_amd/csrc/pw_gemm.hip
--- a/torchok_amd/csrc/pw_gemm.hip
+++ b/torchok_amd/csrc/pw_gemm.hip
@@ -308,6 +308,10 @@
           for (int e = 0; e < 8; ++e) {
             if (!((bits >> e) & 1u)) o[e] = (bf16)0.f;
             s1[half * 8 + e] += bf2f(o[e]);
+          }
+          if (a.e2 != nullptr) {
+#pragma unroll
+            for (int e = 0; e < 8; ++e) s2[half * 8 + e] = fmaf(bf2f(o[e]), bf2f(ev[mt][half][e]), s2[half * 8 + e]);
           }
         }
         stg16(yp + half * 32, o);
diff --git a/torchok_amd/engine/functional.py b/torchok_amd/engine/functional.py
--- a/torchok_amd/engine/functional.py
+++ b/torchok_amd/engine/functional.py
@@ -254,12 +254,14 @@
         self.y = self.mask = None
         self.region = None
         self.fused_partial = None
+        self.dz_stored = False
         self.pool = None
         self.ypool = None
 
     def release(self):
         self.x = self.out = self.shortcut = None
         self.y = self.pk = self.mask = self.fused_partial = self.pool = self.ypool = None
+        self.dz_stored = False
         self.mean = self.rstd = self.scale = self.shift = None
 
     def wants_fused_bwd_stats(self) -> bool:
@@ -267,7 +269,10 @@
                 and (self.act is None or (self.act == RELU and self.mask is not None)))
 
     def _apply_bwd(self, lib, st, g, mask, coef, dy, ds_ptr, ds_acc, m, kp):
-        if self.act in MASKLESS:
+        if self.dz_stored:
+            _C.check(lib.tok_bn_bwd_apply(ptr(g), ptr(self.y), None, ptr(self.scale), ptr(self.shift), ptr(coef), 0, ptr(dy),
+                                          ds_ptr, ds_acc, m, kp, st), 'tok_bn_bwd_apply')
+        elif self.act in MASKLESS:
             bwd_apply, name = _maskless(lib, self.act, 'bwd_apply')
             _C.check(bwd_apply(ptr(g), ptr(self.y), ptr(self.scale), ptr(self.shift), ptr(coef), ptr(dy), m, kp, st), name)
         else:
@@ -358,7 +363,7 @@
                 ds_ptr, ds_acc = None, 0
                 if sc_need:
                     if sc.grad is None and out.grad_owned:
-                        ds_ptr = ptr(g)
+                        ds_ptr = None if self.dz_stored else ptr(g)
                         donate_grad(sc, g)
                     else:
                         tgt, ds_acc = grad_target(sc)
@@ -398,7 +403,14 @@
             partial = _rider_partial(lib, rider, prod, d, x.cp, g.device)
             bn_y = ptr(prod.y) if rider == BN_SUMS else None
             bn_mask = ptr(prod.mask) if (rider == MASKED_DZ or (rider == BN_SUMS and prod.relu)) else None
-            if sub is not None:
+            if rider == BN_SUMS and _stores_dz(lib, prod, d, sub is not None):
+                if sub is not None:
+                    x.grad_sub = None
+                    assert acc == 0
+                _C.check(lib.tok_conv_dgrad_maskstats(d, ptr(dy), ptr(self.pk.dgrad), ptr(tgt), acc, ptr(sub), bn_y, bn_mask,
+                                                      ptr(partial), st), 'tok_conv_dgrad_maskstats')
+                prod.dz_stored = True
+            elif sub is not None:
                 x.grad_sub = None
                 assert acc == 0
                 _C.check(lib.tok_conv_dgrad_subacc(d, ptr(dy), ptr(self.pk.dgrad), ptr(tgt), ptr(sub), bn_y, bn_mask, ptr(partial),
@@ -428,6 +440,19 @@
     return None
 
 
+def _maskstats_entry(lib):
+    return getattr(lib, 'tok_conv_dgrad_maskstats', None)
+
+
+def _stores_dz(lib, prod, d, with_sub: bool) -> bool:
+    if _maskstats_entry(lib) is None:
+        return False
+    sc = prod.shortcut
+    if not (prod.relu and prod.mask is not None and sc is not None and sc.requires_grad):
+        return False
+    return bool(lib.tok_conv_dgrad_maskstats_ok(d, int(with_sub)))
+
+
 def _rider_partial(lib, rider, prod, d, cp: int, dev) -> Optional[torch.Tensor]:
     if rider is None:
         return None
@@ -441,6 +466,21 @@
 
 
 
+def _wgrad2_entry(lib):
+    return getattr(lib, 'tok_conv_wgrad2', None)
+
+
+def _gram_pair_ok(lib, unit, proj) -> bool:
+    if _wgrad2_entry(lib) is None:
+        return False
+    pc, pb = proj.conv, proj.bn
+    if not (pc.weight.requires_grad or proj.x.requires_grad or pb.weight.requires_grad or pb.bias.requires_grad):
+        return False
+    if getattr(proj, 'stream_tag', 0) != getattr(unit, 'stream_tag', 0):
+        return False
+    return bool(lib.tok_conv_wgrad2_ok(unit.desc, proj.desc))
+
+
 FUSE_UNIT3 = os.environ.get('TOK_FUSE_UNIT3', '1') != '0'
 UNIT3_MIN_ROWS = int(os.environ.get('TOK_UNIT3_MIN_ROWS', '100000'))
 
@@ -463,9 +503,10 @@
         self.x = self.out = self.shortcut = self.mask = None
         self.relu = True
         self.masked_partial = None
+        self.gram = None
 
     def release(self):
-        self.x = self.out = self.shortcut = self.mask = self.masked_partial = None
+        self.x = self.out = self.shortcut = self.mask = self.masked_partial = self.gram = None
         self.mean = self.rstd = self.wz = self.zsum = self.pk = None
 
     def backward(self):
@@ -488,11 +529,13 @@
             _C.check(lib.tok_relu_mask_reduce(ptr(g), ptr(self.mask) if self.relu else None, m, kp, ptr(dz), ptr(partial), st),
                      'tok_relu_mask_reduce')
         out.grad = None
+        pair = None
         if sc is not None and sc.requires_grad:
             if donate_grad(sc, dz):
                 scn = sc.node
                 if isinstance(scn, _Unit3Node) and not scn.relu and sc.uses == 1 and scn.masked_partial is None:
                     scn.masked_partial = (partial, rows)
+                    pair = scn
             else:
                 tgt, _ = grad_target(sc)
                 tgt.add_(dz)
@@ -501,7 +544,14 @@
         g_need, b_need = bn.weight.requires_grad, bn.bias.requires_grad
         if not (w_need or x_need or g_need or b_need):
             return
-        G = PG.weight_grad(d, x.data, dz, kp, p)[0]
+        if self.gram is not None:
+            G, self.gram = self.gram, None
+        elif pair is not None and _gram_pair_ok(lib, self, pair):
+            G, pair.gram, gram_ws = PG.weight_grad_pair(d, x.data, pair.desc, pair.x.data, dz)
+            if self.region is not None:
+                self.region.keep_until_join(pair.gram, gram_ws)
+        else:
+            G = PG.weight_grad(d, x.data, dz, kp, p)[0]
         gbuf, bbuf, pacc, finish = PG.pair_sinks(bn.weight if g_need else None, bn.bias if b_need else None)
         dw, wacc = PG.sink(conv.weight) if w_need else (torch.empty((kp, p), dtype=F32, device=dev), 0)
         coef = torch.empty((3, kp), dtype=F32, device=dev)
diff --git a/torchok_amd/engine/paramgrad.py b/torchok_amd/engine/paramgrad.py
--- a/torchok_amd/engine/paramgrad.py
+++ b/torchok_amd/engine/paramgrad.py
@@ -89,6 +89,17 @@
     return dst, ws
 
 
+def weight_grad_pair(d1: _C.ConvDesc, x1: torch.Tensor, d2: _C.ConvDesc, x2: torch.Tensor, dy: torch.Tensor):
+    lib = _C.lib()
+    ws_bytes = lib.tok_conv_wgrad2_ws_bytes(d1, d2)
+    ws = torch.empty(max(ws_bytes // 4, 1), dtype=F32, device=dy.device)
+    g1 = torch.empty((d1.k, d1.c), dtype=F32, device=dy.device)
+    g2 = torch.empty((d2.k, d2.c), dtype=F32, device=dy.device)
+    _C.check(lib.tok_conv_wgrad2(d1, ptr(x1), d2, ptr(x2), ptr(dy), ptr(g1), 0, ptr(g2), 0, ptr(ws), ws_bytes, stream_ptr()),
+             'tok_conv_wgrad2')
+    return g1, g2, ws
+
+
 def colsum(dy: torch.Tensor, m: int, n_pad: int, dst: torch.Tensor, accumulate: int, two_pass: bool, n_real: int = 0):
     lib, st = _C.lib(), stream_ptr()
     if not two_pass:
```

Result: no change. 14580 (median of 6 runs) (+1.0%).
